# ofsoundof/GRL-Image-Restoration

Hardware: NVIDIA H100
Metric: Mpix/s (input pixels) GRL-Base x4 SR 256x256 tiles (higher is better)
Workload: dtype f16

## Files before the change

grl-image-restoration_b200/csrc/gemm_tc.cu:

```cuda
#include <algorithm>

#include "grl_common.cuh"
#include "tc_common.cuh"
#include "ops_tc.h"

namespace grl {
namespace tc {

EncodeTiledFn encode_tiled_fn() {
  static EncodeTiledFn fn = nullptr;
  if (!fn) {
    void* p = nullptr;
    cudaDriverEntryPointQueryResult q;
    if (cudaGetDriverEntryPoint("cuTensorMapEncodeTiled", &p, cudaEnableDefault, &q) == cudaSuccess &&
        q == cudaDriverEntryPointSuccess)
      fn = (EncodeTiledFn)p;
  }
  return fn;
}

__device__ __forceinline__ float gelu_as(float x) {
  const float z = fabsf(x) * 0.70710678118654752440f;
  float t, e;
  asm("rcp.approx.ftz.f32 %0, %1;" : "=f"(t) : "f"(fmaf(0.3275911f, z, 1.0f)));
  asm("ex2.approx.ftz.f32 %0, %1;" : "=f"(e) : "f"(-z * z * 1.4426950408889634f));
  float p = fmaf(1.061405429f, t, -1.453152027f);
  p = fmaf(p, t, 1.421413741f);
  p = fmaf(p, t, -0.284496736f);
  p = fmaf(p, t, 0.254829592f);
  const float erf_abs = fmaf(-p * t, e, 1.0f);
  const float half_x = 0.5f * x;
  return fmaf(half_x, copysignf(erf_abs, x), half_x);
}
__device__ __forceinline__ float tc_act(float v, int act, float slope) {
  if (act == GRL_ACT_GELU) return gelu_as(v);
  if (act == GRL_ACT_LEAKY) return v > 0.f ? v : v * slope;
  return v;
}

constexpr int kStages = 4;
constexpr int kBM = 128, kBK = 64;
constexpr int kTH = 8, kTW = 16;
constexpr int kEpiWarps = 8, kEpiThreads = kEpiWarps * 32, kThreads = kEpiThreads + 32;

__host__ __device__ constexpr int stage_pitch32(int c) { return (c % 8 == 4) ? c : ((c + 3) / 4 * 4 % 8 == 4 ? (c + 3) / 4 * 4 : (c + 3) / 4 * 4 + 4); }

template <int BN>
struct GemmSmem {
  static constexpr int A_BYTES = kBM * kBK * 2;
  static constexpr int B_BYTES = BN * kBK * 2;
  static constexpr int STAGE = A_BYTES + B_BYTES;
  static constexpr int PIPE = kStages * STAGE;
  static constexpr int AP = BN + 4;
  static constexpr int ACC = kBM * AP * 4;
  static constexpr int STG32 = kBM * stage_pitch32(BN <= 192 ? (BN == 192 ? 188 : BN) : 4) * 4;
  static constexpr int STG16 = kBM * (BN + 8) * 2;
  static constexpr int STG = (STG32 > STG16 ? STG32 : STG16);
  static constexpr int OFF_STG = ACC;
  static constexpr int OFF_TOK = ((PIPE > ACC + STG ? PIPE : ACC + STG) + 15) / 16 * 16;
  static constexpr int OFF_PAR = OFF_TOK + 128 * 8 + 128 * 4;
  static constexpr int OFF_MOM = OFF_PAR + 3 * BN * 4;
  static constexpr int OFF_BAR = OFF_MOM + 2 * 128 * 3 * 4;
  static constexpr int TOTAL = OFF_BAR + 128 + 1024 ;
  static_assert(AP % 8 == 4, "accumulator pitch");
  static_assert(TOTAL <= 232448, "shared memory budget");
};

__device__ __forceinline__ void epi_barrier() { asm volatile("bar.sync 1, 256;" ::: "memory"); }

__device__ __forceinline__ void acc_row32(const float* p, uint32_t (&v)[32]) {
#pragma unroll
  for (int j = 0; j < 32; j += 4) {
    const uint4 x = *reinterpret_cast<const uint4*>(p + j);
    v[j] = x.x, v[j + 1] = x.y, v[j + 2] = x.z, v[j + 3] = x.w;
  }
}

template <int BN, int FMT>
__device__ __forceinline__ void mma_loop(float (&acc)[BN / 64][32], uint8_t* smem, uint64_t* full, uint64_t* empty,
                                         int nk_total, int half, int et) {
  using S = GemmSmem<BN>;
  for (int kc = 0; kc < nk_total; ++kc) {
    const int s = kc % kStages;
    mbar_wait(&full[s], (kc / kStages) & 1);
    const uint32_t sa = smem_u32(smem + s * S::STAGE) + half * (64 * 128);
    const uint32_t sb = smem_u32(smem + s * S::STAGE + S::A_BYTES);
    wgmma_fence();
#pragma unroll
    for (int k = 0; k < kBK / 16; ++k) {
      const uint64_t ad = gmma_desc(sa + k * 32, 16, 1024, SWZ_128B);
#pragma unroll
      for (int j = 0; j < BN / 64; ++j) {
        const uint64_t bd = gmma_desc(sb + j * (64 * 128) + k * 32, 16, 1024, SWZ_128B);
        if (FMT == FMT_BF16) wgmma_n64_bf16(acc[j], ad, bd, true);
        else wgmma_n64_f16(acc[j], ad, bd, true);
      }
    }
    wgmma_commit();
    wgmma_wait<1>();
    if (kc > 0 && (et & 127) == 0) mbar_arrive(&empty[(kc - 1) % kStages]);
  }
  wgmma_wait<0>();
}

template <int BN, int EPI, bool CONV>
__global__ void __launch_bounds__(kThreads, 1)
gemm_tc_kernel(const __grid_constant__ CUtensorMap tmA, const __grid_constant__ CUtensorMap tmB, const GemmTcArgs a) {
  extern __shared__ uint8_t smem_raw[];
  uint8_t* smem = reinterpret_cast<uint8_t*>((reinterpret_cast<uintptr_t>(smem_raw) + 1023) & ~uintptr_t(1023));
  using S = GemmSmem<BN>;
  constexpr int AP = S::AP;
  uint64_t* full = reinterpret_cast<uint64_t*>(smem + S::OFF_BAR);
  uint64_t* empty = full + kStages;
  long long* s_tok = reinterpret_cast<long long*>(smem + S::OFF_TOK);
  int* s_img = reinterpret_cast<int*>(smem + S::OFF_TOK + 128 * 8);
  float* s_bias = reinterpret_cast<float*>(smem + S::OFF_PAR);
  float* s_gamma = s_bias + BN;
  float* s_beta = s_gamma + BN;
  float* s_mom = reinterpret_cast<float*>(smem + S::OFF_MOM);
  float* accs = reinterpret_cast<float*>(smem);

  const int warp = threadIdx.x >> 5, lane = threadIdx.x & 31;
  const int n_tiles = a.n_tiles;
  const int m_idx = blockIdx.x / n_tiles;
  const int n0 = (blockIdx.x - m_idx * n_tiles) * BN;
  const int nk_total = a.taps * a.nk;
  int m0 = 0, tb = 0, ty0 = 0, tx0 = 0;
  if (CONV) {
    int t = m_idx;
    const int tx = t % a.tiles_x;
    t /= a.tiles_x;
    const int ty = t % a.tiles_y;
    tb = t / a.tiles_y;
    ty0 = ty * kTH;
    tx0 = tx * kTW;
  } else {
    m0 = m_idx * kBM;
  }

  if (threadIdx.x == 0) {
    for (int s = 0; s < kStages; ++s) {
      mbar_init(&full[s], 1);
      mbar_init(&empty[s], 2);
    }
    mbar_init_fence();
    tma_prefetch_desc(&tmA);
    tma_prefetch_desc(&tmB);
  }
  __syncthreads();

  if (warp == kEpiWarps) {
    if (lane == 0) {
      for (int kc = 0; kc < nk_total; ++kc) {
        const int s = kc % kStages;
        mbar_wait(&empty[s], ((kc / kStages) & 1) ^ 1);
        uint8_t* sa = smem + s * S::STAGE;
        uint8_t* sb = sa + S::A_BYTES;
        mbar_expect_tx(&full[s], S::STAGE);
        if (CONV) {
          const int tap = kc / a.nk, c0 = (kc - tap * a.nk) * kBK;
          tma_load_4d(sa, &tmA, &full[s], c0, tx0 + (tap % 3) - 1, ty0 + (tap / 3) - 1, tb);
        } else {
          tma_load_2d(sa, &tmA, &full[s], kc * kBK, m0);
        }
        tma_load_2d(sb, &tmB, &full[s], kc * kBK, n0);
      }
    }
    return;
  }

  const int et = threadIdx.x;
  const int q = warp & 3;
  const int row = q * 32 + lane;
  const int half = et >> 7;
  const int fmt = a.fmt;
  uint16_t* out16 = reinterpret_cast<uint16_t*>(a.out_bf16);
  {
    long long tok;
    if (CONV) {
      const int y = ty0 + row / kTW, x = tx0 + row % kTW;
      tok = (y < a.H && x < a.W) ? ((long long)tb * a.H + y) * a.W + x : -1;
    } else {
      tok = (long long)m0 + row;
      if (tok >= a.M) tok = -1;
    }
    if (half == 0) {
      s_tok[row] = tok;
      s_img[row] = (EPI == EPI_LN && tok >= 0) ? (int)(tok / a.L) : 0;
    }
    for (int c = et; c < BN; c += kEpiThreads) {
      const int n = n0 + c;
      s_bias[c] = (n < a.N) ? a.bias[n] : 0.f;
      if (EPI == EPI_LN) {
        s_gamma[c] = (c < a.C) ? a.gamma[c] : 0.f;
        s_beta[c] = (c < a.C) ? a.beta[c] : 0.f;
      }
    }
  }
  {
    float acc[BN / 64][32];
#pragma unroll
    for (int j = 0; j < BN / 64; ++j)
#pragma unroll
      for (int e = 0; e < 32; ++e) acc[j][e] = 0.f;
    if (fmt == FMT_BF16) mma_loop<BN, FMT_BF16>(acc, smem, full, empty, nk_total, half, et);
    else mma_loop<BN, FMT_F16>(acc, smem, full, empty, nk_total, half, et);
    epi_barrier();
    const int w = (et >> 5) & 3, r0 = half * 64 + 16 * w + (lane >> 2), cq = 2 * (lane & 3);
#pragma unroll
    for (int j = 0; j < BN / 64; ++j)
#pragma unroll
      for (int i = 0; i < 8; ++i) {
        const int c = j * 64 + 8 * i + cq;
        *reinterpret_cast<float2*>(accs + r0 * AP + c) = make_float2(acc[j][4 * i], acc[j][4 * i + 1]);
        *reinterpret_cast<float2*>(accs + (r0 + 8) * AP + c) = make_float2(acc[j][4 * i + 2], acc[j][4 * i + 3]);
      }
  }
  epi_barrier();
  uint32_t v[32];

    if (EPI == EPI_BIAS_ACT && a.epi_mode == 2) {
      const long long tok = s_tok[row];
      for (int c0 = 32 * half; c0 < BN; c0 += 64) {
        if (n0 + c0 >= a.N) break;
        acc_row32(accs + row * AP + c0, v);
        if (tok < 0) continue;
        float o[32];
#pragma unroll
        for (int j = 0; j < 32; ++j) {
          const int n = n0 + c0 + j;
          float val = tc_act(__uint_as_float(v[j]) + s_bias[c0 + j], a.act, a.slope);
          if (a.res_f32 && n < a.N_f32) val += __ldg(a.res_f32 + tok * a.ldr + n);
          o[j] = (n < a.N) ? val : 0.f;
          if (a.out_f32 && n < a.N_f32) a.out_f32[tok * a.ldo_f32 + n] = o[j];
          if (CONV && a.out_nchw && n < a.N_f32) {
            const int r = a.nchw_r, rr = r * r;
            const int c = n / rr, q = n - c * rr;
            const int yy = (ty0 + row / kTW) * r + q / r, xx = (tx0 + row % kTW) * r + q % r;
            if (yy < a.Hc && xx < a.Wc)
              a.out_nchw[(((long long)tb * (a.N_f32 / rr) + c) * a.Hc + yy) * a.Wc + xx] = fmaf(o[j], a.post_scale, a.post_shift[c & 3]);
          }
        }
        if (out16) {
#pragma unroll
          for (int j = 0; j < 32; j += 8)
            if (n0 + c0 + j < a.ldo_bf16)
              *reinterpret_cast<uint4*>(out16 + tok * a.ldo_bf16 + n0 + c0 + j) =
                  make_uint4(pack16(o[j], o[j + 1], fmt), pack16(o[j + 2], o[j + 3], fmt), pack16(o[j + 4], o[j + 5], fmt),
                             pack16(o[j + 6], o[j + 7], fmt));
        }
      }
    } else if (a.epi_mode == 1) {
      const int Cw = (EPI == EPI_LN) ? a.C : a.N_f32;
      const int pitch = stage_pitch32(Cw);
      float* stg = reinterpret_cast<float*>(smem + S::OFF_STG);
      const bool res_in_stage = a.res_f32 != nullptr;
      if (res_in_stage) {
        const int C4r = Cw >> 2, ewr = et >> 5;
        for (int r = ewr; r < kBM; r += kEpiWarps) {
          const long long rtok = s_tok[r];
          for (int c4 = lane; c4 < C4r; c4 += 32)
            cp_async_16(stg + r * pitch + c4 * 4, a.res_f32 + (rtok >= 0 ? rtok : 0) * a.ldr + c4 * 4, rtok >= 0);
        }
        cp_async_commit();
      }
      if (EPI == EPI_LN) {
        float s1 = 0.f, s2 = 0.f, x0 = 0.f;
        int nh = 0;
        for (int c0 = 32 * half; c0 < Cw; c0 += 64) {
          acc_row32(accs + row * AP + c0, v);
          if (c0 == 32 * half) x0 = __uint_as_float(v[0]) + s_bias[c0];
#pragma unroll
          for (int j = 0; j < 32; ++j)
            if (c0 + j < Cw) {
              const float d = __uint_as_float(v[j]) + s_bias[c0 + j] - x0;
              s1 += d;
              s2 = fmaf(d, d, s2);
              ++nh;
            }
        }
        {
          const float fn = (float)nh;
          const float m1 = nh > 0 ? s1 / fn : 0.f;
          s_mom[(half * kBM + row) * 3 + 0] = x0 + m1;
          s_mom[(half * kBM + row) * 3 + 1] = nh > 0 ? fmaxf(s2 - s1 * m1, 0.f) : 0.f;
          s_mom[(half * kBM + row) * 3 + 2] = fn;
        }
        if (res_in_stage) cp_async_wait<0>();
        epi_barrier();
        float mean, rstd;
        {
          const float m0 = s_mom[row * 3 + 0], q0 = s_mom[row * 3 + 1], c0n = s_mom[row * 3 + 2];
          const float m1 = s_mom[(kBM + row) * 3 + 0], q1 = s_mom[(kBM + row) * 3 + 1], c1n = s_mom[(kBM + row) * 3 + 2];
          const float n = c0n + c1n, d = (c1n > 0.f) ? m1 - m0 : 0.f;
          mean = m0 + d * (c1n / n);
          const float M2 = q0 + q1 + d * d * (c0n * c1n / n);
          rstd = rsqrtf(M2 / n + a.eps);
        }
        for (int c0 = 32 * half; c0 < Cw; c0 += 64) {
          acc_row32(accs + row * AP + c0, v);
#pragma unroll
          for (int j = 0; j < 32; j += 4) {
            if (c0 + j < Cw) {
              float4* sp = reinterpret_cast<float4*>(stg + row * pitch + c0 + j);
              float4 acc4 = res_in_stage ? *sp : make_float4(0.f, 0.f, 0.f, 0.f);
              float o4[4] = {acc4.x, acc4.y, acc4.z, acc4.w};
#pragma unroll
              for (int e = 0; e < 4; ++e) {
                const int c = c0 + j + e;
                o4[e] += ((__uint_as_float(v[j + e]) + s_bias[c] - mean) * rstd * s_gamma[c] + s_beta[c]) * a.res_scale;
              }
              *sp = make_float4(o4[0], o4[1], o4[2], o4[3]);
            }
          }
        }
      } else {
        if (res_in_stage) {
          cp_async_wait<0>();
          epi_barrier();
        }
        for (int c0 = 32 * half; c0 < Cw; c0 += 64) {
          acc_row32(accs + row * AP + c0, v);
#pragma unroll
          for (int j = 0; j < 32; j += 4) {
            if (c0 + j < Cw) {
              float4* sp = reinterpret_cast<float4*>(stg + row * pitch + c0 + j);
              float4 acc4 = res_in_stage ? *sp : make_float4(0.f, 0.f, 0.f, 0.f);
              float o4[4] = {acc4.x, acc4.y, acc4.z, acc4.w};
#pragma unroll
              for (int e = 0; e < 4; ++e) o4[e] += tc_act(__uint_as_float(v[j + e]) + s_bias[c0 + j + e], a.act, a.slope);
              *sp = make_float4(o4[0], o4[1], o4[2], o4[3]);
            }
          }
        }
      }
      epi_barrier();
      const int C4 = Cw >> 2;
      const int P4 = out16 ? (int)(a.ldo_bf16 >> 2) : C4;
      const int ew = et >> 5;
      const bool has_cab = (EPI == EPI_LN) && a.cab_y != nullptr;
      const uint16_t* caby = reinterpret_cast<const uint16_t*>(a.cab_y);
      constexpr int RB = 8;
      for (int cbase = 0; cbase < P4; cbase += 32) {
        const int c4 = cbase + lane;
        const bool col_real = c4 < C4, col_any = c4 < P4;
        for (int rb = 0; rb < kBM / kEpiWarps; rb += RB) {
          long long tok[RB];
          float4 gg[RB];
          uint2 cy[RB];
#pragma unroll
          for (int i = 0; i < RB; ++i) {
            tok[i] = s_tok[ew + kEpiWarps * (rb + i)];
            gg[i] = make_float4(0.f, 0.f, 0.f, 0.f);
            cy[i] = make_uint2(0u, 0u);
            if (tok[i] >= 0 && col_real) {
              if (has_cab) {
                cy[i] = __ldg(reinterpret_cast<const uint2*>(caby + tok[i] * a.ld_caby + c4 * 4));
                gg[i] = __ldg(reinterpret_cast<const float4*>(a.cab_gate + (long long)s_img[ew + kEpiWarps * (rb + i)] * Cw + c4 * 4));
              }
            }
          }
#pragma unroll
          for (int i = 0; i < RB; ++i) {
            if (tok[i] < 0 || !col_any) continue;
            float4 val = make_float4(0.f, 0.f, 0.f, 0.f);
            if (col_real) {
              val = *reinterpret_cast<const float4*>(stg + (ew + kEpiWarps * (rb + i)) * pitch + c4 * 4);
              if (has_cab) {
                const float2 c01 = unpack16(cy[i].x, fmt), c23 = unpack16(cy[i].y, fmt);
                val.x = fmaf(c01.x, gg[i].x, val.x), val.y = fmaf(c01.y, gg[i].y, val.y);
                val.z = fmaf(c23.x, gg[i].z, val.z), val.w = fmaf(c23.y, gg[i].w, val.w);
              }
              if (a.out_f32) *reinterpret_cast<float4*>(a.out_f32 + tok[i] * a.ldo_f32 + c4 * 4) = val;
            }
            if (out16)
              *reinterpret_cast<uint2*>(out16 + tok[i] * a.ldo_bf16 + c4 * 4) =
                  make_uint2(pack16(val.x, val.y, fmt), pack16(val.z, val.w, fmt));
          }
        }
      }
    } else {
      constexpr int P16 = BN + 8;
      uint16_t* stg = reinterpret_cast<uint16_t*>(smem + S::OFF_STG);
      const int ncols = min(BN, a.N - n0);
      for (int c0 = 32 * half; c0 < ncols; c0 += 64) {
        acc_row32(accs + row * AP + c0, v);
        float o[32];
        if (EPI == EPI_QKV) {
          const int slot = (n0 + c0) >> 5;
          float ss = 0.f;
#pragma unroll
          for (int j = 0; j < 32; ++j) {
            o[j] = __uint_as_float(v[j]) + s_bias[c0 + j];
            ss = fmaf(o[j], o[j], ss);
          }
          const float sc = __ldg(a.slot_scale + slot);
          const float mul = sc > 0.f ? sc * rsqrtf(fmaxf(ss, 1e-24f)) : 1.0f;
#pragma unroll
          for (int j = 0; j < 32; ++j) o[j] *= mul;
        } else {
#pragma unroll
          for (int j = 0; j < 32; ++j) o[j] = tc_act(__uint_as_float(v[j]) + s_bias[c0 + j], a.act, a.slope);
        }
#pragma unroll
        for (int j = 0; j < 32; j += 8)
          *reinterpret_cast<uint4*>(stg + row * P16 + c0 + j) =
              make_uint4(pack16(o[j], o[j + 1], fmt), pack16(o[j + 2], o[j + 3], fmt), pack16(o[j + 4], o[j + 5], fmt),
                         pack16(o[j + 6], o[j + 7], fmt));
      }
      epi_barrier();
      const int nvec = min((long long)ncols, a.ldo_bf16 - n0) >> 3;
      const int ew = et >> 5;
      if (CONV && a.ps_r > 0) {
        const int ps = a.ps_r, Cq = a.N / (ps * ps);
        const int nv = min(BN, a.N - n0) >> 3;
#pragma unroll 4
        for (int r = ew; r < kBM; r += kEpiWarps) {
          if (s_tok[r] < 0) continue;
          const int y = ty0 + r / kTW, x = tx0 + r % kTW;
          for (int vv = lane; vv < nv; vv += 32) {
            const int n = n0 + vv * 8;
            const int q = n / Cq, c = n - q * Cq;
            const long long dtok = ((long long)tb * a.H * ps + y * ps + q / ps) * ((long long)a.W * ps) + x * ps + q % ps;
            *reinterpret_cast<uint4*>(out16 + dtok * a.ldo_bf16 + c) = *reinterpret_cast<const uint4*>(stg + r * P16 + vv * 8);
          }
        }
      } else {
#pragma unroll 4
        for (int r = ew; r < kBM; r += kEpiWarps) {
          const long long tok = s_tok[r];
          if (tok < 0) continue;
          for (int vv = lane; vv < nvec; vv += 32)
            *reinterpret_cast<uint4*>(out16 + tok * a.ldo_bf16 + n0 + vv * 8) = *reinterpret_cast<const uint4*>(stg + r * P16 + vv * 8);
        }
      }
    }

}

static int make_map(CUtensorMap* m, const void* base, int rank, const cuuint64_t* dims, const cuuint64_t* strides_bytes,
                    const cuuint32_t* box, int fmt) {
  EncodeTiledFn fn = encode_tiled_fn();
  if (!fn) return fail(GRL_ERR_CUDA, "cuTensorMapEncodeTiled is not available from the driver");
  cuuint32_t ones[5] = {1, 1, 1, 1, 1};
  CUresult rc = fn(m, fmt == FMT_BF16 ? CU_TENSOR_MAP_DATA_TYPE_BFLOAT16 : CU_TENSOR_MAP_DATA_TYPE_FLOAT16, (cuuint32_t)rank, const_cast<void*>(base), dims, strides_bytes,
                   box, ones, CU_TENSOR_MAP_INTERLEAVE_NONE, CU_TENSOR_MAP_SWIZZLE_128B,
                   CU_TENSOR_MAP_L2_PROMOTION_L2_128B, CU_TENSOR_MAP_FLOAT_OOB_FILL_NONE);
  if (rc != CUDA_SUCCESS) return fail(GRL_ERR_CUDA, "cuTensorMapEncodeTiled failed with CUresult %d", (int)rc);
  return GRL_OK;
}

template <int BN, int EPI, bool CONV>
static int launch_one(const CUtensorMap& tmA, const CUtensorMap& tmB, const GemmTcArgs& a, dim3 grid, cudaStream_t st) {
  auto kern = gemm_tc_kernel<BN, EPI, CONV>;
  static bool configured[kMaxDevices] = {false};
  int dev = 0;
  GRL_CUDA(cudaGetDevice(&dev));
  if (dev < 0 || dev >= kMaxDevices || !configured[dev]) {
    GRL_CUDA(cudaFuncSetAttribute(kern, cudaFuncAttributeMaxDynamicSharedMemorySize, GemmSmem<BN>::TOTAL));
    if (dev >= 0 && dev < kMaxDevices) configured[dev] = true;
  }
  kern<<<grid, kThreads, GemmSmem<BN>::TOTAL, st>>>(tmA, tmB, a);
  GRL_LAUNCH_CHECK("gemm_tc_kernel");
  return GRL_OK;
}

template <int EPI, bool CONV>
static int dispatch_bn(int bn, const CUtensorMap& tmA, const CUtensorMap& tmB, const GemmTcArgs& a, dim3 grid,
                       cudaStream_t st) {
  switch (bn) {
    case 64: return launch_one<64, EPI, CONV>(tmA, tmB, a, grid, st);
    case 128: return launch_one<128, EPI, CONV>(tmA, tmB, a, grid, st);
    case 192: return launch_one<192, EPI, CONV>(tmA, tmB, a, grid, st);
    case 256: return launch_one<256, EPI, CONV>(tmA, tmB, a, grid, st);
  }
  return fail(GRL_ERR_INVALID, "gemm_tc: unsupported tile width %d", bn);
}

int pick_bn(int npad) {
  if (npad <= 64) return 64;
  if (npad <= 128) return 128;
  if (npad % 192 == 0 || npad <= 192) return 192;
  if (npad % 256 == 0) return 256;
  return npad % 128 == 0 ? 128 : 192;
}

int plan_gemm_tc(const GemmTcProblem& p, GemmTcArgs& a, int* bn_out) {
  GRL_REQUIRE(p.kpad % kBK == 0 && p.kpad > 0, "gemm_tc: K pad %d must be a multiple of 64", p.kpad);
  GRL_REQUIRE(p.npad % 32 == 0 && p.npad > 0, "gemm_tc: N pad %d must be a multiple of 32", p.npad);
  int bn = (p.epi == EPI_LN) ? (p.npad <= 64 ? 64 : p.npad <= 128 ? 128 : p.npad <= 192 ? 192 : 256) : pick_bn(p.npad);
  GRL_REQUIRE(p.epi != EPI_LN || p.npad <= 256, "gemm_tc: LayerNorm epilogue needs the whole row in one tile (N=%d)",
              p.npad);
  const bool conv = p.taps == 9;
  if (a.ps_r > 0)
    GRL_REQUIRE(conv && p.epi == EPI_BIAS_ACT && !a.out_f32 && !a.res_f32 && a.out_bf16 && a.N % (a.ps_r * a.ps_r) == 0 &&
                    (a.N / (a.ps_r * a.ps_r)) % 8 == 0 && a.ldo_bf16 >= a.N / (a.ps_r * a.ps_r),
                "gemm_tc: pixel-shuffle store needs a 16-bit-only conv epilogue with N %% r^2 == 0 and N / r^2 %% 8 == 0");
  if (a.out_nchw)
    GRL_REQUIRE(conv && p.epi == EPI_BIAS_ACT && a.nchw_r >= 1 && a.N_f32 % (a.nchw_r * a.nchw_r) == 0 &&
                    a.N_f32 / (a.nchw_r * a.nchw_r) <= 4 && a.Hc > 0 && a.Wc > 0,
                "gemm_tc: NCHW tail store needs a conv with <= 4 output channels");
  GRL_REQUIRE(p.taps == 1 || p.taps == 9, "gemm_tc: taps must be 1 or 9");
  a.epi_mode = 0;
  if (p.epi == EPI_LN || (p.epi == EPI_BIAS_ACT && (a.out_f32 || a.res_f32))) {
    const int cw = p.epi == EPI_LN ? a.C : a.N_f32;
    const int cap = bn == 64 ? GemmSmem<64>::STG : bn == 128 ? GemmSmem<128>::STG : bn == 192 ? GemmSmem<192>::STG
                                                                                               : GemmSmem<256>::STG;
    const bool ok = p.npad <= bn && cw > 0 && cw % 4 == 0 && kBM * stage_pitch32(cw) * 4 <= cap &&
                    (!a.out_f32 || a.ldo_f32 % 4 == 0) && (!a.res_f32 || a.ldr % 4 == 0) &&
                    (!a.out_bf16 || a.ldo_bf16 % 4 == 0);
    GRL_REQUIRE(ok || p.epi != EPI_LN, "gemm_tc: LayerNorm epilogue needs C %% 4 == 0 and C <= 188 (got %d)", cw);
    a.epi_mode = ok ? 1 : 2;
  }
  if (a.out_nchw) a.epi_mode = 2;
  GRL_REQUIRE(p.epi == EPI_BIAS_ACT || p.epi == EPI_QKV || p.epi == EPI_LN, "gemm_tc: unknown epilogue %d", p.epi);
  GRL_REQUIRE(!conv || p.epi == EPI_BIAS_ACT, "gemm_tc: %s epilogue is linear-only", p.epi == EPI_QKV ? "QKV" : "LN");
  a.nk = p.kpad / kBK;
  a.taps = p.taps;
  a.n_tiles = ceil_div(p.npad, bn);
  if (conv) {
    a.H = p.H, a.W = p.W;
    a.tiles_x = ceil_div(p.W, kTW), a.tiles_y = ceil_div(p.H, kTH);
    a.M = (long long)p.B * p.H * p.W;
    GRL_REQUIRE((long long)a.tiles_x * a.tiles_y * p.B * a.n_tiles < (1ll << 31), "gemm_tc: grid too large");
    a.total_tiles = a.tiles_x * a.tiles_y * p.B * a.n_tiles;
  } else {
    a.M = p.M;
    GRL_REQUIRE((long long)ceil_div(p.M, kBM) * a.n_tiles < (1ll << 31), "gemm_tc: grid too large");
    a.total_tiles = (int)(ceil_div(p.M, kBM) * a.n_tiles);
  }
  *bn_out = bn;
  return GRL_OK;
}

int launch_gemm_tc(const GemmTcProblem& p, GemmTcArgs a, cudaStream_t st) {
  int bn = 0, rc;
  if ((rc = plan_gemm_tc(p, a, &bn)) != GRL_OK) return rc;
  if (a.M == 0) return GRL_OK;
  CUtensorMap tmA, tmB;
  if (p.taps == 9) {
    cuuint64_t dims[4] = {(cuuint64_t)p.kpad, (cuuint64_t)p.W, (cuuint64_t)p.H, (cuuint64_t)p.B};
    cuuint64_t str[3] = {(cuuint64_t)p.kpad * 2, (cuuint64_t)p.W * p.kpad * 2, (cuuint64_t)p.H * p.W * p.kpad * 2};
    cuuint32_t box[4] = {(cuuint32_t)kBK, (cuuint32_t)kTW, (cuuint32_t)kTH, 1};
    if ((rc = make_map(&tmA, p.x, 4, dims, str, box, a.fmt)) != GRL_OK) return rc;
  } else {
    cuuint64_t dims[2] = {(cuuint64_t)p.kpad, (cuuint64_t)p.M};
    cuuint64_t str[1] = {(cuuint64_t)p.kpad * 2};
    cuuint32_t box[2] = {(cuuint32_t)kBK, (cuuint32_t)kBM};
    if ((rc = make_map(&tmA, p.x, 2, dims, str, box, a.fmt)) != GRL_OK) return rc;
  }
  {
    cuuint64_t dims[2] = {(cuuint64_t)p.kpad * p.taps, (cuuint64_t)p.npad};
    cuuint64_t str[1] = {(cuuint64_t)p.kpad * p.taps * 2};
    cuuint32_t box[2] = {(cuuint32_t)kBK, (cuuint32_t)bn};
    if ((rc = make_map(&tmB, p.w, 2, dims, str, box, a.fmt)) != GRL_OK) return rc;
  }
  const dim3 grid((unsigned)a.total_tiles);
  switch (p.epi) {
    case EPI_QKV: return dispatch_bn<EPI_QKV, false>(bn, tmA, tmB, a, grid, st);
    case EPI_LN: return dispatch_bn<EPI_LN, false>(bn, tmA, tmB, a, grid, st);
  }
  return p.taps == 9 ? dispatch_bn<EPI_BIAS_ACT, true>(bn, tmA, tmB, a, grid, st)
                     : dispatch_bn<EPI_BIAS_ACT, false>(bn, tmA, tmB, a, grid, st);
}

}
}
```

grl-image-restoration_b200/csrc/tc_common.cuh:

```cuda
#pragma once
#include <cuda.h>
#include <cuda_bf16.h>
#include <cuda_fp16.h>
#include <cuda_runtime.h>
#include <stdint.h>

namespace grl {
namespace tc {

__device__ __forceinline__ uint32_t smem_u32(const void* p) { return (uint32_t)__cvta_generic_to_shared(p); }

__device__ __forceinline__ void mbar_init(uint64_t* bar, uint32_t count) {
  asm volatile("mbarrier.init.shared::cta.b64 [%0], %1;" ::"r"(smem_u32(bar)), "r"(count) : "memory");
}
__device__ __forceinline__ void mbar_init_fence() { asm volatile("fence.mbarrier_init.release.cluster;" ::: "memory"); }
__device__ __forceinline__ void mbar_expect_tx(uint64_t* bar, uint32_t bytes) {
  asm volatile("mbarrier.arrive.expect_tx.shared::cta.b64 _, [%0], %1;" ::"r"(smem_u32(bar)), "r"(bytes) : "memory");
}
__device__ __forceinline__ void mbar_arrive(uint64_t* bar) {
  asm volatile("mbarrier.arrive.shared::cta.b64 _, [%0];" ::"r"(smem_u32(bar)) : "memory");
}
__device__ __forceinline__ bool mbar_try_wait(uint64_t* bar, uint32_t parity) {
  uint32_t ok;
  asm volatile(
      "{\n\t.reg .pred p;\n\t"
      "mbarrier.try_wait.parity.shared::cta.b64 p, [%1], %2, %3;\n\t"
      "selp.u32 %0, 1, 0, p;\n\t}"
      : "=r"(ok)
      : "r"(smem_u32(bar)), "r"(parity), "r"(1000000u)
      : "memory");
  return ok != 0;
}
__device__ __forceinline__ void mbar_wait(uint64_t* bar, uint32_t parity) {
  if (mbar_try_wait(bar, parity)) return;
  int spins = 0;
  long long t0 = 0;
  while (!mbar_try_wait(bar, parity)) {
    if ((++spins & 63) == 0) {
      const long long now = clock64();
      if (t0 == 0) t0 = now;
      else if (now - t0 > 4000000000ll) __trap();
    }
  }
}

__device__ __forceinline__ void fence_proxy_async_smem() { asm volatile("fence.proxy.async.shared::cta;" ::: "memory"); }

__device__ __forceinline__ void tma_prefetch_desc(const CUtensorMap* m) {
  asm volatile("prefetch.tensormap [%0];" ::"l"(reinterpret_cast<uint64_t>(m)) : "memory");
}
__device__ __forceinline__ void tma_load_2d(void* smem, const CUtensorMap* m, uint64_t* bar, int c0, int c1) {
  asm volatile(
      "cp.async.bulk.tensor.2d.shared::cluster.global.mbarrier::complete_tx::bytes [%0], [%1, {%3, %4}], [%2];" ::"r"(
          smem_u32(smem)),
      "l"(reinterpret_cast<uint64_t>(m)), "r"(smem_u32(bar)), "r"(c0), "r"(c1)
      : "memory");
}
__device__ __forceinline__ void tma_load_4d(void* smem, const CUtensorMap* m, uint64_t* bar, int c0, int c1, int c2,
                                            int c3) {
  asm volatile(
      "cp.async.bulk.tensor.4d.shared::cluster.global.mbarrier::complete_tx::bytes [%0], [%1, {%3, %4, %5, %6}], "
      "[%2];" ::"r"(smem_u32(smem)),
      "l"(reinterpret_cast<uint64_t>(m)), "r"(smem_u32(bar)), "r"(c0), "r"(c1), "r"(c2), "r"(c3)
      : "memory");
}

__device__ __forceinline__ void cp_async_16(void* smem, const void* gmem, bool valid) {
  const int sz = valid ? 16 : 0;
  asm volatile("cp.async.cg.shared.global [%0], [%1], 16, %2;" ::"r"(smem_u32(smem)), "l"(gmem), "r"(sz) : "memory");
}
__device__ __forceinline__ void bulk_load_1d(void* smem, const void* gmem, uint32_t bytes, uint64_t* bar) {
  asm volatile("cp.async.bulk.shared::cluster.global.mbarrier::complete_tx::bytes [%0], [%1], %2, [%3];" ::"r"(smem_u32(smem)),
               "l"(gmem), "r"(bytes), "r"(smem_u32(bar))
               : "memory");
}
__device__ __forceinline__ void cp_async_commit() { asm volatile("cp.async.commit_group;" ::: "memory"); }
template <int N>
__device__ __forceinline__ void cp_async_wait() {
  asm volatile("cp.async.wait_group %0;" ::"n"(N) : "memory");
}

enum : uint32_t { SWZ_NONE = 0, SWZ_128B = 1, SWZ_64B = 2, SWZ_32B = 3 };
__device__ __forceinline__ uint64_t gmma_desc(uint32_t saddr, uint32_t lbo_bytes, uint32_t sbo_bytes, uint32_t swz) {
  uint64_t d = 0;
  d |= (uint64_t)((saddr & 0x3FFFFu) >> 4);
  d |= (uint64_t)((lbo_bytes >> 4) & 0x3FFFu) << 16;
  d |= (uint64_t)((sbo_bytes >> 4) & 0x3FFFu) << 32;
  d |= (uint64_t)swz << 62;
  return d;
}
__device__ __forceinline__ void wgmma_fence() { asm volatile("wgmma.fence.sync.aligned;" ::: "memory"); }
__device__ __forceinline__ void wgmma_commit() { asm volatile("wgmma.commit_group.sync.aligned;" ::: "memory"); }
template <int N>
__device__ __forceinline__ void wgmma_wait() {
  asm volatile("wgmma.wait_group.sync.aligned %0;" ::"n"(N) : "memory");
}
template <int N>
__device__ __forceinline__ void wgmma_fence_regs(float (&d)[N]) {
#pragma unroll
  for (int i = 0; i < N; ++i) asm volatile("" : "+f"(d[i])::"memory");
}
#define GRL_D16 "+f"(d[0]), "+f"(d[1]), "+f"(d[2]), "+f"(d[3]), "+f"(d[4]), "+f"(d[5]), "+f"(d[6]), "+f"(d[7]), "+f"(d[8]), "+f"(d[9]), "+f"(d[10]), "+f"(d[11]), "+f"(d[12]), "+f"(d[13]), "+f"(d[14]), "+f"(d[15])
#define GRL_D32 GRL_D16, "+f"(d[16]), "+f"(d[17]), "+f"(d[18]), "+f"(d[19]), "+f"(d[20]), "+f"(d[21]), "+f"(d[22]), "+f"(d[23]), "+f"(d[24]), "+f"(d[25]), "+f"(d[26]), "+f"(d[27]), "+f"(d[28]), "+f"(d[29]), "+f"(d[30]), "+f"(d[31])
#define GRL_R16 "%0, %1, %2, %3, %4, %5, %6, %7, %8, %9, %10, %11, %12, %13, %14, %15"
#define GRL_R32 GRL_R16 ", %16, %17, %18, %19, %20, %21, %22, %23, %24, %25, %26, %27, %28, %29, %30, %31"
#define GRL_WGMMA(NAME, N, NREG, REGS, OUTS, A, B, P, TY, TNSPB)                                                    \
  __device__ __forceinline__ void NAME(float (&d)[NREG], uint64_t adesc, uint64_t bdesc, bool accumulate) {         \
    asm volatile("{\n\t.reg .pred p;\n\tsetp.ne.b32 p, %" #P ", 0;\n\t"                                                 \
                 "wgmma.mma_async.sync.aligned.m64n" #N "k16.f32." TY "." TY " {" REGS "}, %" #A ", %" #B ", p, 1, 1, 0, " \
                 #TNSPB ";\n\t}"                                                                                     \
                 : OUTS                                                                                              \
                 : "l"(adesc), "l"(bdesc), "r"((uint32_t)accumulate));                                               \
  }
GRL_WGMMA(wgmma_n64_bf16, 64, 32, GRL_R32, GRL_D32, 32, 33, 34, "bf16", 0)
GRL_WGMMA(wgmma_n64_f16, 64, 32, GRL_R32, GRL_D32, 32, 33, 34, "f16", 0)
GRL_WGMMA(wgmma_n32t_bf16, 32, 16, GRL_R16, GRL_D16, 16, 17, 18, "bf16", 1)
GRL_WGMMA(wgmma_n32t_f16, 32, 16, GRL_R16, GRL_D16, 16, 17, 18, "f16", 1)
#define GRL_WGMMA_RS(NAME, TY)                                                                                        \
  __device__ __forceinline__ void NAME(float (&d)[16], const uint32_t (&a)[4], uint64_t bdesc) {                     \
    asm volatile("{\n\t.reg .pred p;\n\tsetp.ne.b32 p, 1, 0;\n\t"                                                    \
                 "wgmma.mma_async.sync.aligned.m64n32k16.f32." TY "." TY " {" GRL_R16 "}, {%16, %17, %18, %19}, %20, " \
                 "p, 1, 1, 1;\n\t}"                                                                                 \
                 : GRL_D16                                                                                          \
                 : "r"(a[0]), "r"(a[1]), "r"(a[2]), "r"(a[3]), "l"(bdesc));                                         \
  }
GRL_WGMMA_RS(wgmma_rs_n32t_bf16, "bf16")
GRL_WGMMA_RS(wgmma_rs_n32t_f16, "f16")

__device__ __forceinline__ uint32_t pack_bf16(float lo, float hi) {
  __nv_bfloat162 v = __floats2bfloat162_rn(lo, hi);
  return *reinterpret_cast<uint32_t*>(&v);
}
enum : int { FMT_F16 = 0, FMT_BF16 = 1 };
__device__ __forceinline__ uint32_t pack_f16(float lo, float hi) {
  uint32_t d;
  asm("cvt.rn.satfinite.f16x2.f32 %0, %1, %2;" : "=r"(d) : "f"(hi), "f"(lo));
  return d;
}
__device__ __forceinline__ uint32_t pack16(float lo, float hi, int fmt) {
  return fmt == FMT_BF16 ? pack_bf16(lo, hi) : pack_f16(lo, hi);
}
__device__ __forceinline__ float2 unpack16(uint32_t v, int fmt) {
  if (fmt == FMT_BF16) return make_float2(__uint_as_float(v << 16), __uint_as_float(v & 0xFFFF0000u));
  return __half22float2(*reinterpret_cast<const __half2*>(&v));
}
__device__ __forceinline__ float unpack16_one(uint16_t v, int fmt) {
  if (fmt == FMT_BF16) return __uint_as_float((uint32_t)v << 16);
  return __half2float(*reinterpret_cast<const __half*>(&v));
}

typedef CUresult (*EncodeTiledFn)(CUtensorMap*, CUtensorMapDataType, cuuint32_t, void*, const cuuint64_t*,
                                  const cuuint64_t*, const cuuint32_t*, const cuuint32_t*, CUtensorMapInterleave,
                                  CUtensorMapSwizzle, CUtensorMapL2promotion, CUtensorMapFloatOOBfill);
EncodeTiledFn encode_tiled_fn();

}
}
```

Before: 1.576.

## Make tensor-core GEMM persistent with wide WGMMA and register-resident epilogue

Turns the warp-specialized TMA/WGMMA GEMM into a persistent kernel that loops over tiles with a global pipeline iteration counter, so loads for the next tile overlap the current tile's epilogue. Single wide m64nBNk16 WGMMA instructions (N=128/192/256) replace multiple n64 issues. The epilogue works directly from registers instead of staging the fp32 accumulator tile through shared memory, and computes LayerNorm statistics with warp shuffles and Chan merging. The freed shared memory allows per-BN stage counts, cp.async prefetch of the residual and two CTAs per SM for BN=64. The risks are higher register pressure from the wide accumulators and more complex barrier phase tracking.

Measured after the change: 1.627 (median of 6 runs). 1.03x the previous value.

```diff
diff --git a/grl-image-restoration_b200/csrc/gemm_tc.cu b/grl-image-restoration_b200/csrc/gemm_tc.cu
--- a/grl-image-restoration_b200/csrc/gemm_tc.cu
+++ b/grl-image-restoration_b200/csrc/gemm_tc.cu
@@ -38,7 +38,6 @@
   return v;
 }
 
-constexpr int kStages = 4;
 constexpr int kBM = 128, kBK = 64;
 constexpr int kTH = 8, kTW = 16;
 constexpr int kEpiWarps = 8, kEpiThreads = kEpiWarps * 32, kThreads = kEpiThreads + 32;
@@ -47,99 +46,132 @@
 
 template <int BN>
 struct GemmSmem {
+  static constexpr int STAGES = (BN >= 192 || BN == 64) ? 3 : 4;
   static constexpr int A_BYTES = kBM * kBK * 2;
   static constexpr int B_BYTES = BN * kBK * 2;
   static constexpr int STAGE = A_BYTES + B_BYTES;
-  static constexpr int PIPE = kStages * STAGE;
-  static constexpr int AP = BN + 4;
-  static constexpr int ACC = kBM * AP * 4;
+  static constexpr int PIPE = STAGES * STAGE;
   static constexpr int STG32 = kBM * stage_pitch32(BN <= 192 ? (BN == 192 ? 188 : BN) : 4) * 4;
   static constexpr int STG16 = kBM * (BN + 8) * 2;
   static constexpr int STG = (STG32 > STG16 ? STG32 : STG16);
-  static constexpr int OFF_STG = ACC;
-  static constexpr int OFF_TOK = ((PIPE > ACC + STG ? PIPE : ACC + STG) + 15) / 16 * 16;
+  static constexpr int OFF_STG = PIPE;
+  static constexpr int OFF_TOK = OFF_STG + STG;
   static constexpr int OFF_PAR = OFF_TOK + 128 * 8 + 128 * 4;
-  static constexpr int OFF_MOM = OFF_PAR + 3 * BN * 4;
-  static constexpr int OFF_BAR = OFF_MOM + 2 * 128 * 3 * 4;
-  static constexpr int TOTAL = OFF_BAR + 128 + 1024 ;
-  static_assert(AP % 8 == 4, "accumulator pitch");
+  static constexpr int OFF_BAR = OFF_PAR + 3 * BN * 4;
+  static constexpr int TOTAL = OFF_BAR + 2 * STAGES * 8 + 1024 ;
+  static_assert(STG % 16 == 0, "staging alignment");
   static_assert(TOTAL <= 232448, "shared memory budget");
 };
 
 __device__ __forceinline__ void epi_barrier() { asm volatile("bar.sync 1, 256;" ::: "memory"); }
 
-__device__ __forceinline__ void acc_row32(const float* p, uint32_t (&v)[32]) {
-#pragma unroll
-  for (int j = 0; j < 32; j += 4) {
-    const uint4 x = *reinterpret_cast<const uint4*>(p + j);
-    v[j] = x.x, v[j + 1] = x.y, v[j + 2] = x.z, v[j + 3] = x.w;
-  }
+struct TileCoord {
+  int n0, m0, tb, ty0, tx0;
+};
+template <int BN, bool CONV>
+__device__ __forceinline__ TileCoord tile_coord(const GemmTcArgs& a, int tile) {
+  TileCoord t{};
+  const int m_idx = tile / a.n_tiles;
+  t.n0 = (tile - m_idx * a.n_tiles) * BN;
+  if (CONV) {
+    int u = m_idx;
+    const int tx = u % a.tiles_x;
+    u /= a.tiles_x;
+    const int ty = u % a.tiles_y;
+    t.tb = u / a.tiles_y;
+    t.ty0 = ty * kTH;
+    t.tx0 = tx * kTW;
+  } else {
+    t.m0 = m_idx * kBM;
+  }
+  return t;
+}
+template <bool CONV>
+__device__ __forceinline__ long long row_token(const GemmTcArgs& a, const TileCoord& t, int r) {
+  if (CONV) {
+    const int y = t.ty0 + r / kTW, x = t.tx0 + r % kTW;
+    return (y < a.H && x < a.W) ? ((long long)t.tb * a.H + y) * a.W + x : -1;
+  }
+  const long long tok = (long long)t.m0 + r;
+  return tok < a.M ? tok : -1;
+}
+
+__device__ __forceinline__ void chan_merge(float& m0, float& q0, float& n0, float m1, float q1, float n1) {
+  if (n1 > 0.f) {
+    const float n = n0 + n1, d = m1 - m0;
+    m0 = m0 + d * (n1 / n);
+    q0 = q0 + q1 + d * d * (n0 * n1 / n);
+    n0 = n;
+  }
+}
+
+template <int BN>
+__device__ __forceinline__ void wgmma_wide_f16(float (&d)[BN / 64][32], uint64_t ad, uint64_t bd) {
+  if constexpr (BN == 128) wgmma_n128_f16(d, ad, bd);
+  else if constexpr (BN == 192) wgmma_n192_f16(d, ad, bd);
+  else if constexpr (BN == 256) wgmma_n256_f16(d, ad, bd);
+}
+template <int BN>
+__device__ __forceinline__ void wgmma_wide_bf16(float (&d)[BN / 64][32], uint64_t ad, uint64_t bd) {
+  if constexpr (BN == 128) wgmma_n128_bf16(d, ad, bd);
+  else if constexpr (BN == 192) wgmma_n192_bf16(d, ad, bd);
+  else if constexpr (BN == 256) wgmma_n256_bf16(d, ad, bd);
 }
 
 template <int BN, int FMT>
 __device__ __forceinline__ void mma_loop(float (&acc)[BN / 64][32], uint8_t* smem, uint64_t* full, uint64_t* empty,
-                                         int nk_total, int half, int et) {
+                                         uint32_t it, int nk_total, int half, int et) {
   using S = GemmSmem<BN>;
   for (int kc = 0; kc < nk_total; ++kc) {
-    const int s = kc % kStages;
-    mbar_wait(&full[s], (kc / kStages) & 1);
+    const uint32_t g = it + kc;
+    const int s = g % S::STAGES;
+    mbar_wait(&full[s], (g / S::STAGES) & 1);
     const uint32_t sa = smem_u32(smem + s * S::STAGE) + half * (64 * 128);
     const uint32_t sb = smem_u32(smem + s * S::STAGE + S::A_BYTES);
     wgmma_fence();
 #pragma unroll
     for (int k = 0; k < kBK / 16; ++k) {
       const uint64_t ad = gmma_desc(sa + k * 32, 16, 1024, SWZ_128B);
-#pragma unroll
-      for (int j = 0; j < BN / 64; ++j) {
-        const uint64_t bd = gmma_desc(sb + j * (64 * 128) + k * 32, 16, 1024, SWZ_128B);
-        if (FMT == FMT_BF16) wgmma_n64_bf16(acc[j], ad, bd, true);
-        else wgmma_n64_f16(acc[j], ad, bd, true);
+      const uint64_t bd = gmma_desc(sb + k * 32, 16, 1024, SWZ_128B);
+      if (BN == 64) {
+        if (FMT == FMT_BF16) wgmma_n64_bf16(acc[0], ad, bd, true);
+        else wgmma_n64_f16(acc[0], ad, bd, true);
+      } else if (FMT == FMT_BF16) {
+        wgmma_wide_bf16<BN>(acc, ad, bd);
+      } else {
+        wgmma_wide_f16<BN>(acc, ad, bd);
       }
     }
     wgmma_commit();
     wgmma_wait<1>();
-    if (kc > 0 && (et & 127) == 0) mbar_arrive(&empty[(kc - 1) % kStages]);
+    if (kc > 0 && (et & 127) == 0) mbar_arrive(&empty[(g - 1) % S::STAGES]);
   }
   wgmma_wait<0>();
+  if ((et & 127) == 0) mbar_arrive(&empty[(it + nk_total - 1) % S::STAGES]);
+#pragma unroll
+  for (int j = 0; j < BN / 64; ++j) wgmma_fence_regs(acc[j]);
 }
 
 template <int BN, int EPI, bool CONV>
-__global__ void __launch_bounds__(kThreads, 1)
+__global__ void __launch_bounds__(kThreads, (BN == 64 && EPI != EPI_LN) ? 2 : 1)
 gemm_tc_kernel(const __grid_constant__ CUtensorMap tmA, const __grid_constant__ CUtensorMap tmB, const GemmTcArgs a) {
   extern __shared__ uint8_t smem_raw[];
   uint8_t* smem = reinterpret_cast<uint8_t*>((reinterpret_cast<uintptr_t>(smem_raw) + 1023) & ~uintptr_t(1023));
   using S = GemmSmem<BN>;
-  constexpr int AP = S::AP;
+  constexpr int NS = S::STAGES;
   uint64_t* full = reinterpret_cast<uint64_t*>(smem + S::OFF_BAR);
-  uint64_t* empty = full + kStages;
+  uint64_t* empty = full + NS;
   long long* s_tok = reinterpret_cast<long long*>(smem + S::OFF_TOK);
   int* s_img = reinterpret_cast<int*>(smem + S::OFF_TOK + 128 * 8);
   float* s_bias = reinterpret_cast<float*>(smem + S::OFF_PAR);
   float* s_gamma = s_bias + BN;
   float* s_beta = s_gamma + BN;
-  float* s_mom = reinterpret_cast<float*>(smem + S::OFF_MOM);
-  float* accs = reinterpret_cast<float*>(smem);
 
   const int warp = threadIdx.x >> 5, lane = threadIdx.x & 31;
-  const int n_tiles = a.n_tiles;
-  const int m_idx = blockIdx.x / n_tiles;
-  const int n0 = (blockIdx.x - m_idx * n_tiles) * BN;
   const int nk_total = a.taps * a.nk;
-  int m0 = 0, tb = 0, ty0 = 0, tx0 = 0;
-  if (CONV) {
-    int t = m_idx;
-    const int tx = t % a.tiles_x;
-    t /= a.tiles_x;
-    const int ty = t % a.tiles_y;
-    tb = t / a.tiles_y;
-    ty0 = ty * kTH;
-    tx0 = tx * kTW;
-  } else {
-    m0 = m_idx * kBM;
-  }
 
   if (threadIdx.x == 0) {
-    for (int s = 0; s < kStages; ++s) {
+    for (int s = 0; s < NS; ++s) {
       mbar_init(&full[s], 1);
       mbar_init(&empty[s], 2);
     }
@@ -147,192 +179,191 @@
     tma_prefetch_desc(&tmA);
     tma_prefetch_desc(&tmB);
   }
+  if (EPI == EPI_LN)
+    for (int c = threadIdx.x; c < BN; c += kThreads) {
+      s_gamma[c] = (c < a.C) ? a.gamma[c] : 0.f;
+      s_beta[c] = (c < a.C) ? a.beta[c] : 0.f;
+    }
   __syncthreads();
 
   if (warp == kEpiWarps) {
     if (lane == 0) {
-      for (int kc = 0; kc < nk_total; ++kc) {
-        const int s = kc % kStages;
-        mbar_wait(&empty[s], ((kc / kStages) & 1) ^ 1);
-        uint8_t* sa = smem + s * S::STAGE;
-        uint8_t* sb = sa + S::A_BYTES;
-        mbar_expect_tx(&full[s], S::STAGE);
-        if (CONV) {
-          const int tap = kc / a.nk, c0 = (kc - tap * a.nk) * kBK;
-          tma_load_4d(sa, &tmA, &full[s], c0, tx0 + (tap % 3) - 1, ty0 + (tap / 3) - 1, tb);
-        } else {
-          tma_load_2d(sa, &tmA, &full[s], kc * kBK, m0);
+      uint32_t it = 0;
+      for (int tile = blockIdx.x; tile < a.total_tiles; tile += gridDim.x) {
+        const TileCoord t = tile_coord<BN, CONV>(a, tile);
+        for (int kc = 0; kc < nk_total; ++kc, ++it) {
+          const int s = it % NS;
+          mbar_wait(&empty[s], ((it / NS) & 1) ^ 1);
+          uint8_t* sa = smem + s * S::STAGE;
+          uint8_t* sb = sa + S::A_BYTES;
+          mbar_expect_tx(&full[s], S::STAGE);
+          if (CONV) {
+            const int tap = kc / a.nk, c0 = (kc - tap * a.nk) * kBK;
+            tma_load_4d(sa, &tmA, &full[s], c0, t.tx0 + (tap % 3) - 1, t.ty0 + (tap / 3) - 1, t.tb);
+          } else {
+            tma_load_2d(sa, &tmA, &full[s], kc * kBK, t.m0);
+          }
+          tma_load_2d(sb, &tmB, &full[s], kc * kBK, t.n0);
         }
-        tma_load_2d(sb, &tmB, &full[s], kc * kBK, n0);
       }
     }
     return;
   }
 
   const int et = threadIdx.x;
-  const int q = warp & 3;
-  const int row = q * 32 + lane;
   const int half = et >> 7;
+  const int rA = half * 64 + 16 * ((et >> 5) & 3) + (lane >> 2), cq = 2 * (lane & 3);
   const int fmt = a.fmt;
   uint16_t* out16 = reinterpret_cast<uint16_t*>(a.out_bf16);
-  {
-    long long tok;
-    if (CONV) {
-      const int y = ty0 + row / kTW, x = tx0 + row % kTW;
-      tok = (y < a.H && x < a.W) ? ((long long)tb * a.H + y) * a.W + x : -1;
-    } else {
-      tok = (long long)m0 + row;
-      if (tok >= a.M) tok = -1;
-    }
-    if (half == 0) {
-      s_tok[row] = tok;
-      s_img[row] = (EPI == EPI_LN && tok >= 0) ? (int)(tok / a.L) : 0;
-    }
-    for (int c = et; c < BN; c += kEpiThreads) {
-      const int n = n0 + c;
-      s_bias[c] = (n < a.N) ? a.bias[n] : 0.f;
+  const int Cw = (EPI == EPI_LN) ? a.C : a.N_f32;
+  const int pitch = stage_pitch32(Cw);
+  const bool res_in_stage = a.epi_mode == 1 && a.res_f32 != nullptr;
+  float* stg32 = reinterpret_cast<float*>(smem + S::OFF_STG);
+  constexpr int P16 = BN + 8;
+  uint16_t* stg16 = reinterpret_cast<uint16_t*>(smem + S::OFF_STG);
+  uint32_t it = 0;
+  int bias_n0 = -1;
+
+  for (int tile = blockIdx.x; tile < a.total_tiles; tile += gridDim.x, it += nk_total) {
+    const TileCoord t = tile_coord<BN, CONV>(a, tile);
+    if (et < kBM) {
+      const long long tok = row_token<CONV>(a, t, et);
+      s_tok[et] = tok;
+      s_img[et] = (EPI == EPI_LN && tok >= 0) ? (int)(tok / a.L) : 0;
+    }
+    if (t.n0 != bias_n0) {
+      for (int c = et; c < BN; c += kEpiThreads) s_bias[c] = (t.n0 + c < a.N) ? a.bias[t.n0 + c] : 0.f;
+      bias_n0 = t.n0;
+    }
+    if (res_in_stage) {
+      const int C4r = Cw >> 2;
+      for (int r = et >> 5; r < kBM; r += kEpiWarps) {
+        const long long rtok = row_token<CONV>(a, t, r);
+        for (int c4 = lane; c4 < C4r; c4 += 32)
+          cp_async_16(stg32 + r * pitch + c4 * 4, a.res_f32 + (rtok >= 0 ? rtok : 0) * a.ldr + c4 * 4, rtok >= 0);
+      }
+      cp_async_commit();
+    }
+    float acc[BN / 64][32];
+#pragma unroll
+    for (int j = 0; j < BN / 64; ++j)
+#pragma unroll
+      for (int e = 0; e < 32; ++e) acc[j][e] = 0.f;
+    if (fmt == FMT_BF16) mma_loop<BN, FMT_BF16>(acc, smem, full, empty, it, nk_total, half, et);
+    else mma_loop<BN, FMT_F16>(acc, smem, full, empty, it, nk_total, half, et);
+    if (res_in_stage) cp_async_wait<0>();
+    epi_barrier();
+
+    if (BN <= 192 && EPI == EPI_BIAS_ACT && a.epi_mode == 2) {
+      long long tokr[2] = {row_token<CONV>(a, t, rA), row_token<CONV>(a, t, rA + 8)};
+#pragma unroll
+      for (int j = 0; j < BN / 64; ++j)
+#pragma unroll
+        for (int i = 0; i < 8; ++i) {
+          const int c = 64 * j + 8 * i + cq;
+          if (t.n0 + (c & ~31) >= a.N) continue;
+#pragma unroll
+          for (int h = 0; h < 2; ++h) {
+            const long long tok = tokr[h];
+            if (tok < 0) continue;
+            const int row = rA + 8 * h;
+            float o[2];
+#pragma unroll
+            for (int e = 0; e < 2; ++e) {
+              const int n = t.n0 + c + e;
+              float val = tc_act(acc[j][4 * i + 2 * h + e] + s_bias[c + e], a.act, a.slope);
+              if (a.res_f32 && n < a.N_f32) val += __ldg(a.res_f32 + tok * a.ldr + n);
+              o[e] = (n < a.N) ? val : 0.f;
+              if (a.out_f32 && n < a.N_f32) a.out_f32[tok * a.ldo_f32 + n] = o[e];
+              if (CONV && a.out_nchw && n < a.N_f32) {
+                const int r = a.nchw_r, rr = r * r;
+                const int ch = n / rr, q = n - ch * rr;
+                const int yy = (t.ty0 + row / kTW) * r + q / r, xx = (t.tx0 + row % kTW) * r + q % r;
+                if (yy < a.Hc && xx < a.Wc)
+                  a.out_nchw[(((long long)t.tb * (a.N_f32 / rr) + ch) * a.Hc + yy) * a.Wc + xx] =
+                      fmaf(o[e], a.post_scale, a.post_shift[ch & 3]);
+              }
+            }
+            if (out16 && t.n0 + (c & ~7) < a.ldo_bf16)
+              *reinterpret_cast<uint32_t*>(out16 + tok * a.ldo_bf16 + t.n0 + c) = pack16(o[0], o[1], fmt);
+          }
+        }
+      epi_barrier();
+      continue;
+    }
+    if (BN <= 192 && a.epi_mode == 1) {
       if (EPI == EPI_LN) {
-        s_gamma[c] = (c < a.C) ? a.gamma[c] : 0.f;
-        s_beta[c] = (c < a.C) ? a.beta[c] : 0.f;
-      }
-    }
-  }
-  {
-    float acc[BN / 64][32];
-#pragma unroll
-    for (int j = 0; j < BN / 64; ++j)
-#pragma unroll
-      for (int e = 0; e < 32; ++e) acc[j][e] = 0.f;
-    if (fmt == FMT_BF16) mma_loop<BN, FMT_BF16>(acc, smem, full, empty, nk_total, half, et);
-    else mma_loop<BN, FMT_F16>(acc, smem, full, empty, nk_total, half, et);
-    epi_barrier();
-    const int w = (et >> 5) & 3, r0 = half * 64 + 16 * w + (lane >> 2), cq = 2 * (lane & 3);
-#pragma unroll
-    for (int j = 0; j < BN / 64; ++j)
-#pragma unroll
-      for (int i = 0; i < 8; ++i) {
-        const int c = j * 64 + 8 * i + cq;
-        *reinterpret_cast<float2*>(accs + r0 * AP + c) = make_float2(acc[j][4 * i], acc[j][4 * i + 1]);
-        *reinterpret_cast<float2*>(accs + (r0 + 8) * AP + c) = make_float2(acc[j][4 * i + 2], acc[j][4 * i + 3]);
-      }
-  }
-  epi_barrier();
-  uint32_t v[32];
-
-    if (EPI == EPI_BIAS_ACT && a.epi_mode == 2) {
-      const long long tok = s_tok[row];
-      for (int c0 = 32 * half; c0 < BN; c0 += 64) {
-        if (n0 + c0 >= a.N) break;
-        acc_row32(accs + row * AP + c0, v);
-        if (tok < 0) continue;
-        float o[32];
-#pragma unroll
-        for (int j = 0; j < 32; ++j) {
-          const int n = n0 + c0 + j;
-          float val = tc_act(__uint_as_float(v[j]) + s_bias[c0 + j], a.act, a.slope);
-          if (a.res_f32 && n < a.N_f32) val += __ldg(a.res_f32 + tok * a.ldr + n);
-          o[j] = (n < a.N) ? val : 0.f;
-          if (a.out_f32 && n < a.N_f32) a.out_f32[tok * a.ldo_f32 + n] = o[j];
-          if (CONV && a.out_nchw && n < a.N_f32) {
-            const int r = a.nchw_r, rr = r * r;
-            const int c = n / rr, q = n - c * rr;
-            const int yy = (ty0 + row / kTW) * r + q / r, xx = (tx0 + row % kTW) * r + q % r;
-            if (yy < a.Hc && xx < a.Wc)
-              a.out_nchw[(((long long)tb * (a.N_f32 / rr) + c) * a.Hc + yy) * a.Wc + xx] = fmaf(o[j], a.post_scale, a.post_shift[c & 3]);
-          }
+        float mean[2], rstd[2];
+#pragma unroll
+        for (int h = 0; h < 2; ++h) {
+          const float x0 = acc[0][2 * h] + s_bias[cq];
+          float s1 = 0.f, s2 = 0.f;
+          int nh = 0;
+#pragma unroll
+          for (int j = 0; j < BN / 64; ++j)
+#pragma unroll
+            for (int i = 0; i < 8; ++i)
+#pragma unroll
+              for (int e = 0; e < 2; ++e) {
+                const int c = 64 * j + 8 * i + cq + e;
+                if (c < Cw) {
+                  const float d = acc[j][4 * i + 2 * h + e] + s_bias[c] - x0;
+                  s1 += d;
+                  s2 = fmaf(d, d, s2);
+                  ++nh;
+                }
+              }
+          float n = (float)nh;
+          const float m1 = nh > 0 ? s1 / n : 0.f;
+          float m = nh > 0 ? x0 + m1 : 0.f;
+          float q = nh > 0 ? fmaxf(s2 - s1 * m1, 0.f) : 0.f;
+#pragma unroll
+          for (int x = 1; x <= 2; x <<= 1) {
+            const float mo = __shfl_xor_sync(0xffffffffu, m, x), qo = __shfl_xor_sync(0xffffffffu, q, x),
+                        no = __shfl_xor_sync(0xffffffffu, n, x);
+            if (lane & x) {
+              float m2 = mo, q2 = qo, n2 = no;
+              chan_merge(m2, q2, n2, m, q, n);
+              m = m2, q = q2, n = n2;
+            } else {
+              chan_merge(m, q, n, mo, qo, no);
+            }
+          }
+          mean[h] = m;
+          rstd[h] = rsqrtf(q / n + a.eps);
         }
-        if (out16) {
-#pragma unroll
-          for (int j = 0; j < 32; j += 8)
-            if (n0 + c0 + j < a.ldo_bf16)
-              *reinterpret_cast<uint4*>(out16 + tok * a.ldo_bf16 + n0 + c0 + j) =
-                  make_uint4(pack16(o[j], o[j + 1], fmt), pack16(o[j + 2], o[j + 3], fmt), pack16(o[j + 4], o[j + 5], fmt),
-                             pack16(o[j + 6], o[j + 7], fmt));
-        }
-      }
-    } else if (a.epi_mode == 1) {
-      const int Cw = (EPI == EPI_LN) ? a.C : a.N_f32;
-      const int pitch = stage_pitch32(Cw);
-      float* stg = reinterpret_cast<float*>(smem + S::OFF_STG);
-      const bool res_in_stage = a.res_f32 != nullptr;
-      if (res_in_stage) {
-        const int C4r = Cw >> 2, ewr = et >> 5;
-        for (int r = ewr; r < kBM; r += kEpiWarps) {
-          const long long rtok = s_tok[r];
-          for (int c4 = lane; c4 < C4r; c4 += 32)
-            cp_async_16(stg + r * pitch + c4 * 4, a.res_f32 + (rtok >= 0 ? rtok : 0) * a.ldr + c4 * 4, rtok >= 0);
-        }
-        cp_async_commit();
-      }
-      if (EPI == EPI_LN) {
-        float s1 = 0.f, s2 = 0.f, x0 = 0.f;
-        int nh = 0;
-        for (int c0 = 32 * half; c0 < Cw; c0 += 64) {
-          acc_row32(accs + row * AP + c0, v);
-          if (c0 == 32 * half) x0 = __uint_as_float(v[0]) + s_bias[c0];
-#pragma unroll
-          for (int j = 0; j < 32; ++j)
-            if (c0 + j < Cw) {
-              const float d = __uint_as_float(v[j]) + s_bias[c0 + j] - x0;
-              s1 += d;
-              s2 = fmaf(d, d, s2);
-              ++nh;
+#pragma unroll
+        for (int j = 0; j < BN / 64; ++j)
+#pragma unroll
+          for (int i = 0; i < 8; ++i) {
+            const int c = 64 * j + 8 * i + cq;
+            if (c >= Cw) continue;
+#pragma unroll
+            for (int h = 0; h < 2; ++h) {
+              float2* sp = reinterpret_cast<float2*>(stg32 + (rA + 8 * h) * pitch + c);
+              float2 o = res_in_stage ? *sp : make_float2(0.f, 0.f);
+              o.x += ((acc[j][4 * i + 2 * h] + s_bias[c] - mean[h]) * rstd[h] * s_gamma[c] + s_beta[c]) * a.res_scale;
+              o.y += ((acc[j][4 * i + 2 * h + 1] + s_bias[c + 1] - mean[h]) * rstd[h] * s_gamma[c + 1] + s_beta[c + 1]) *
+                     a.res_scale;
+              *sp = o;
             }
-        }
-        {
-          const float fn = (float)nh;
-          const float m1 = nh > 0 ? s1 / fn : 0.f;
-          s_mom[(half * kBM + row) * 3 + 0] = x0 + m1;
-          s_mom[(half * kBM + row) * 3 + 1] = nh > 0 ? fmaxf(s2 - s1 * m1, 0.f) : 0.f;
-          s_mom[(half * kBM + row) * 3 + 2] = fn;
-        }
-        if (res_in_stage) cp_async_wait<0>();
-        epi_barrier();
-        float mean, rstd;
-        {
-          const float m0 = s_mom[row * 3 + 0], q0 = s_mom[row * 3 + 1], c0n = s_mom[row * 3 + 2];
-          const float m1 = s_mom[(kBM + row) * 3 + 0], q1 = s_mom[(kBM + row) * 3 + 1], c1n = s_mom[(kBM + row) * 3 + 2];
-          const float n = c0n + c1n, d = (c1n > 0.f) ? m1 - m0 : 0.f;
-          mean = m0 + d * (c1n / n);
-          const float M2 = q0 + q1 + d * d * (c0n * c1n / n);
-          rstd = rsqrtf(M2 / n + a.eps);
-        }
-        for (int c0 = 32 * half; c0 < Cw; c0 += 64) {
-          acc_row32(accs + row * AP + c0, v);
-#pragma unroll
-          for (int j = 0; j < 32; j += 4) {
-            if (c0 + j < Cw) {
-              float4* sp = reinterpret_cast<float4*>(stg + row * pitch + c0 + j);
-              float4 acc4 = res_in_stage ? *sp : make_float4(0.f, 0.f, 0.f, 0.f);
-              float o4[4] = {acc4.x, acc4.y, acc4.z, acc4.w};
-#pragma unroll
-              for (int e = 0; e < 4; ++e) {
-                const int c = c0 + j + e;
-                o4[e] += ((__uint_as_float(v[j + e]) + s_bias[c] - mean) * rstd * s_gamma[c] + s_beta[c]) * a.res_scale;
-              }
-              *sp = make_float4(o4[0], o4[1], o4[2], o4[3]);
+          }
+      } else {
+#pragma unroll
+        for (int j = 0; j < BN / 64; ++j)
+#pragma unroll
+          for (int i = 0; i < 8; ++i) {
+            const int c = 64 * j + 8 * i + cq;
+            if (c >= Cw) continue;
+#pragma unroll
+            for (int h = 0; h < 2; ++h) {
+              float2* sp = reinterpret_cast<float2*>(stg32 + (rA + 8 * h) * pitch + c);
+              float2 o = res_in_stage ? *sp : make_float2(0.f, 0.f);
+              o.x += tc_act(acc[j][4 * i + 2 * h] + s_bias[c], a.act, a.slope);
+              o.y += tc_act(acc[j][4 * i + 2 * h + 1] + s_bias[c + 1], a.act, a.slope);
+              *sp = o;
             }
           }
-        }
-      } else {
-        if (res_in_stage) {
-          cp_async_wait<0>();
-          epi_barrier();
-        }
-        for (int c0 = 32 * half; c0 < Cw; c0 += 64) {
-          acc_row32(accs + row * AP + c0, v);
-#pragma unroll
-          for (int j = 0; j < 32; j += 4) {
-            if (c0 + j < Cw) {
-              float4* sp = reinterpret_cast<float4*>(stg + row * pitch + c0 + j);
-              float4 acc4 = res_in_stage ? *sp : make_float4(0.f, 0.f, 0.f, 0.f);
-              float o4[4] = {acc4.x, acc4.y, acc4.z, acc4.w};
-#pragma unroll
-              for (int e = 0; e < 4; ++e) o4[e] += tc_act(__uint_as_float(v[j + e]) + s_bias[c0 + j + e], a.act, a.slope);
-              *sp = make_float4(o4[0], o4[1], o4[2], o4[3]);
-            }
-          }
-        }
       }
       epi_barrier();
       const int C4 = Cw >> 2;
@@ -365,7 +396,7 @@
             if (tok[i] < 0 || !col_any) continue;
             float4 val = make_float4(0.f, 0.f, 0.f, 0.f);
             if (col_real) {
-              val = *reinterpret_cast<const float4*>(stg + (ew + kEpiWarps * (rb + i)) * pitch + c4 * 4);
+              val = *reinterpret_cast<const float4*>(stg32 + (ew + kEpiWarps * (rb + i)) * pitch + c4 * 4);
               if (has_cab) {
                 const float2 c01 = unpack16(cy[i].x, fmt), c23 = unpack16(cy[i].y, fmt);
                 val.x = fmaf(c01.x, gg[i].x, val.x), val.y = fmaf(c01.y, gg[i].y, val.y);
@@ -380,49 +411,59 @@
         }
       }
     } else {
-      constexpr int P16 = BN + 8;
-      uint16_t* stg = reinterpret_cast<uint16_t*>(smem + S::OFF_STG);
-      const int ncols = min(BN, a.N - n0);
-      for (int c0 = 32 * half; c0 < ncols; c0 += 64) {
-        acc_row32(accs + row * AP + c0, v);
-        float o[32];
-        if (EPI == EPI_QKV) {
-          const int slot = (n0 + c0) >> 5;
-          float ss = 0.f;
-#pragma unroll
-          for (int j = 0; j < 32; ++j) {
-            o[j] = __uint_as_float(v[j]) + s_bias[c0 + j];
-            ss = fmaf(o[j], o[j], ss);
-          }
-          const float sc = __ldg(a.slot_scale + slot);
-          const float mul = sc > 0.f ? sc * rsqrtf(fmaxf(ss, 1e-24f)) : 1.0f;
-#pragma unroll
-          for (int j = 0; j < 32; ++j) o[j] *= mul;
-        } else {
-#pragma unroll
-          for (int j = 0; j < 32; ++j) o[j] = tc_act(__uint_as_float(v[j]) + s_bias[c0 + j], a.act, a.slope);
+      const int ncols = min(BN, a.N - t.n0);
+#pragma unroll
+      for (int j = 0; j < BN / 64; ++j)
+#pragma unroll
+        for (int s32 = 0; s32 < 2; ++s32) {
+          const int c0 = 64 * j + 32 * s32;
+          if (c0 >= ncols) continue;
+          float o[2][8];
+#pragma unroll
+          for (int h = 0; h < 2; ++h)
+#pragma unroll
+            for (int ii = 0; ii < 4; ++ii)
+#pragma unroll
+              for (int e = 0; e < 2; ++e) {
+                const float v = acc[j][4 * (4 * s32 + ii) + 2 * h + e] + s_bias[c0 + 8 * ii + cq + e];
+                o[h][2 * ii + e] = (EPI == EPI_QKV) ? v : tc_act(v, a.act, a.slope);
+              }
+          if (EPI == EPI_QKV) {
+            const float sc = __ldg(a.slot_scale + ((t.n0 + c0) >> 5));
+#pragma unroll
+            for (int h = 0; h < 2; ++h) {
+              float ss = 0.f;
+#pragma unroll
+              for (int k = 0; k < 8; ++k) ss = fmaf(o[h][k], o[h][k], ss);
+              ss += __shfl_xor_sync(0xffffffffu, ss, 1);
+              ss += __shfl_xor_sync(0xffffffffu, ss, 2);
+              const float mul = sc > 0.f ? sc * rsqrtf(fmaxf(ss, 1e-24f)) : 1.0f;
+#pragma unroll
+              for (int k = 0; k < 8; ++k) o[h][k] *= mul;
+            }
+          }
+#pragma unroll
+          for (int h = 0; h < 2; ++h)
+#pragma unroll
+            for (int ii = 0; ii < 4; ++ii)
+              *reinterpret_cast<uint32_t*>(stg16 + (rA + 8 * h) * P16 + c0 + 8 * ii + cq) =
+                  pack16(o[h][2 * ii], o[h][2 * ii + 1], fmt);
         }
-#pragma unroll
-        for (int j = 0; j < 32; j += 8)
-          *reinterpret_cast<uint4*>(stg + row * P16 + c0 + j) =
-              make_uint4(pack16(o[j], o[j + 1], fmt), pack16(o[j + 2], o[j + 3], fmt), pack16(o[j + 4], o[j + 5], fmt),
-                         pack16(o[j + 6], o[j + 7], fmt));
-      }
       epi_barrier();
-      const int nvec = min((long long)ncols, a.ldo_bf16 - n0) >> 3;
+      const int nvec = min((long long)ncols, a.ldo_bf16 - t.n0) >> 3;
       const int ew = et >> 5;
       if (CONV && a.ps_r > 0) {
         const int ps = a.ps_r, Cq = a.N / (ps * ps);
-        const int nv = min(BN, a.N - n0) >> 3;
+        const int nv = ncols >> 3;
 #pragma unroll 4
         for (int r = ew; r < kBM; r += kEpiWarps) {
           if (s_tok[r] < 0) continue;
-          const int y = ty0 + r / kTW, x = tx0 + r % kTW;
+          const int y = t.ty0 + r / kTW, x = t.tx0 + r % kTW;
           for (int vv = lane; vv < nv; vv += 32) {
-            const int n = n0 + vv * 8;
+            const int n = t.n0 + vv * 8;
             const int q = n / Cq, c = n - q * Cq;
-            const long long dtok = ((long long)tb * a.H * ps + y * ps + q / ps) * ((long long)a.W * ps) + x * ps + q % ps;
-            *reinterpret_cast<uint4*>(out16 + dtok * a.ldo_bf16 + c) = *reinterpret_cast<const uint4*>(stg + r * P16 + vv * 8);
+            const long long dtok = ((long long)t.tb * a.H * ps + y * ps + q / ps) * ((long long)a.W * ps) + x * ps + q % ps;
+            *reinterpret_cast<uint4*>(out16 + dtok * a.ldo_bf16 + c) = *reinterpret_cast<const uint4*>(stg16 + r * P16 + vv * 8);
           }
         }
       } else {
@@ -431,11 +472,12 @@
           const long long tok = s_tok[r];
           if (tok < 0) continue;
           for (int vv = lane; vv < nvec; vv += 32)
-            *reinterpret_cast<uint4*>(out16 + tok * a.ldo_bf16 + n0 + vv * 8) = *reinterpret_cast<const uint4*>(stg + r * P16 + vv * 8);
+            *reinterpret_cast<uint4*>(out16 + tok * a.ldo_bf16 + t.n0 + vv * 8) = *reinterpret_cast<const uint4*>(stg16 + r * P16 + vv * 8);
         }
       }
     }
-
+    epi_barrier();
+  }
 }
 
 static int make_map(CUtensorMap* m, const void* base, int rank, const cuuint64_t* dims, const cuuint64_t* strides_bytes,
@@ -450,29 +492,43 @@
   return GRL_OK;
 }
 
+static int sm_count(int dev) {
+  static int sms[kMaxDevices] = {0};
+  if (dev >= 0 && dev < kMaxDevices && sms[dev] > 0) return sms[dev];
+  int n = 0;
+  if (cudaDeviceGetAttribute(&n, cudaDevAttrMultiProcessorCount, dev) != cudaSuccess || n <= 0) return 0;
+  if (dev >= 0 && dev < kMaxDevices) sms[dev] = n;
+  return n;
+}
+
 template <int BN, int EPI, bool CONV>
-static int launch_one(const CUtensorMap& tmA, const CUtensorMap& tmB, const GemmTcArgs& a, dim3 grid, cudaStream_t st) {
+static int launch_one(const CUtensorMap& tmA, const CUtensorMap& tmB, const GemmTcArgs& a, cudaStream_t st) {
   auto kern = gemm_tc_kernel<BN, EPI, CONV>;
-  static bool configured[kMaxDevices] = {false};
+  static int resident[kMaxDevices] = {0};
   int dev = 0;
   GRL_CUDA(cudaGetDevice(&dev));
-  if (dev < 0 || dev >= kMaxDevices || !configured[dev]) {
+  int per_sm = (dev >= 0 && dev < kMaxDevices) ? resident[dev] : 0;
+  if (per_sm == 0) {
     GRL_CUDA(cudaFuncSetAttribute(kern, cudaFuncAttributeMaxDynamicSharedMemorySize, GemmSmem<BN>::TOTAL));
-    if (dev >= 0 && dev < kMaxDevices) configured[dev] = true;
-  }
+    GRL_CUDA(cudaOccupancyMaxActiveBlocksPerMultiprocessor(&per_sm, kern, kThreads, GemmSmem<BN>::TOTAL));
+    if (per_sm <= 0) return fail(GRL_ERR_CUDA, "gemm_tc: kernel does not fit on an SM of device %d", dev);
+    if (dev >= 0 && dev < kMaxDevices) resident[dev] = per_sm;
+  }
+  const int sms = sm_count(dev);
+  if (sms <= 0) return fail(GRL_ERR_CUDA, "gemm_tc: cannot read the SM count of device %d", dev);
+  const dim3 grid((unsigned)std::min((long long)a.total_tiles, (long long)sms * per_sm));
   kern<<<grid, kThreads, GemmSmem<BN>::TOTAL, st>>>(tmA, tmB, a);
   GRL_LAUNCH_CHECK("gemm_tc_kernel");
   return GRL_OK;
 }
 
 template <int EPI, bool CONV>
-static int dispatch_bn(int bn, const CUtensorMap& tmA, const CUtensorMap& tmB, const GemmTcArgs& a, dim3 grid,
-                       cudaStream_t st) {
+static int dispatch_bn(int bn, const CUtensorMap& tmA, const CUtensorMap& tmB, const GemmTcArgs& a, cudaStream_t st) {
   switch (bn) {
-    case 64: return launch_one<64, EPI, CONV>(tmA, tmB, a, grid, st);
-    case 128: return launch_one<128, EPI, CONV>(tmA, tmB, a, grid, st);
-    case 192: return launch_one<192, EPI, CONV>(tmA, tmB, a, grid, st);
-    case 256: return launch_one<256, EPI, CONV>(tmA, tmB, a, grid, st);
+    case 64: return launch_one<64, EPI, CONV>(tmA, tmB, a, st);
+    case 128: return launch_one<128, EPI, CONV>(tmA, tmB, a, st);
+    case 192: return launch_one<192, EPI, CONV>(tmA, tmB, a, st);
+    case 256: return launch_one<256, EPI, CONV>(tmA, tmB, a, st);
   }
   return fail(GRL_ERR_INVALID, "gemm_tc: unsupported tile width %d", bn);
 }
@@ -488,9 +544,10 @@
 int plan_gemm_tc(const GemmTcProblem& p, GemmTcArgs& a, int* bn_out) {
   GRL_REQUIRE(p.kpad % kBK == 0 && p.kpad > 0, "gemm_tc: K pad %d must be a multiple of 64", p.kpad);
   GRL_REQUIRE(p.npad % 32 == 0 && p.npad > 0, "gemm_tc: N pad %d must be a multiple of 32", p.npad);
-  int bn = (p.epi == EPI_LN) ? (p.npad <= 64 ? 64 : p.npad <= 128 ? 128 : p.npad <= 192 ? 192 : 256) : pick_bn(p.npad);
-  GRL_REQUIRE(p.epi != EPI_LN || p.npad <= 256, "gemm_tc: LayerNorm epilogue needs the whole row in one tile (N=%d)",
+  int bn = (p.epi == EPI_LN) ? (p.npad <= 64 ? 64 : p.npad <= 128 ? 128 : 192) : pick_bn(p.npad);
+  GRL_REQUIRE(p.epi != EPI_LN || p.npad <= 192, "gemm_tc: LayerNorm epilogue needs the whole row in one tile (N=%d)",
               p.npad);
+  if (bn == 256 && p.epi == EPI_BIAS_ACT && (a.out_f32 || a.res_f32 || a.out_nchw)) bn = 128;
   const bool conv = p.taps == 9;
   if (a.ps_r > 0)
     GRL_REQUIRE(conv && p.epi == EPI_BIAS_ACT && !a.out_f32 && !a.res_f32 && a.out_bf16 && a.N % (a.ps_r * a.ps_r) == 0 &&
@@ -555,14 +612,13 @@
     cuuint32_t box[2] = {(cuuint32_t)kBK, (cuuint32_t)bn};
     if ((rc = make_map(&tmB, p.w, 2, dims, str, box, a.fmt)) != GRL_OK) return rc;
   }
-  const dim3 grid((unsigned)a.total_tiles);
   switch (p.epi) {
-    case EPI_QKV: return dispatch_bn<EPI_QKV, false>(bn, tmA, tmB, a, grid, st);
-    case EPI_LN: return dispatch_bn<EPI_LN, false>(bn, tmA, tmB, a, grid, st);
-  }
-  return p.taps == 9 ? dispatch_bn<EPI_BIAS_ACT, true>(bn, tmA, tmB, a, grid, st)
-                     : dispatch_bn<EPI_BIAS_ACT, false>(bn, tmA, tmB, a, grid, st);
-}
-
-}
-}
+    case EPI_QKV: return dispatch_bn<EPI_QKV, false>(bn, tmA, tmB, a, st);
+    case EPI_LN: return dispatch_bn<EPI_LN, false>(bn, tmA, tmB, a, st);
+  }
+  return p.taps == 9 ? dispatch_bn<EPI_BIAS_ACT, true>(bn, tmA, tmB, a, st)
+                     : dispatch_bn<EPI_BIAS_ACT, false>(bn, tmA, tmB, a, st);
+}
+
+}
+}
diff --git a/grl-image-restoration_b200/csrc/tc_common.cuh b/grl-image-restoration_b200/csrc/tc_common.cuh
--- a/grl-image-restoration_b200/csrc/tc_common.cuh
+++ b/grl-image-restoration_b200/csrc/tc_common.cuh
@@ -124,6 +124,36 @@
                  : GRL_D16                                                                                          \
                  : "r"(a[0]), "r"(a[1]), "r"(a[2]), "r"(a[3]), "l"(bdesc));                                         \
   }
+__device__ __forceinline__ void wgmma_n128_f16(float (&d)[2][32], uint64_t adesc, uint64_t bdesc) {
+  asm volatile("{\n\t.reg .pred p;\n\tsetp.ne.b32 p, 1, 0;\n\twgmma.mma_async.sync.aligned.m64n128k16.f32.f16.f16 {%0, %1, %2, %3, %4, %5, %6, %7, %8, %9, %10, %11, %12, %13, %14, %15, %16, %17, %18, %19, %20, %21, %22, %23, %24, %25, %26, %27, %28, %29, %30, %31, %32, %33, %34, %35, %36, %37, %38, %39, %40, %41, %42, %43, %44, %45, %46, %47, %48, %49, %50, %51, %52, %53, %54, %55, %56, %57, %58, %59, %60, %61, %62, %63}, %64, %65, p, 1, 1, 0, 0;\n\t}"
+               : "+f"(d[0][0]), "+f"(d[0][1]), "+f"(d[0][2]), "+f"(d[0][3]), "+f"(d[0][4]), "+f"(d[0][5]), "+f"(d[0][6]), "+f"(d[0][7]), "+f"(d[0][8]), "+f"(d[0][9]), "+f"(d[0][10]), "+f"(d[0][11]), "+f"(d[0][12]), "+f"(d[0][13]), "+f"(d[0][14]), "+f"(d[0][15]), "+f"(d[0][16]), "+f"(d[0][17]), "+f"(d[0][18]), "+f"(d[0][19]), "+f"(d[0][20]), "+f"(d[0][21]), "+f"(d[0][22]), "+f"(d[0][23]), "+f"(d[0][24]), "+f"(d[0][25]), "+f"(d[0][26]), "+f"(d[0][27]), "+f"(d[0][28]), "+f"(d[0][29]), "+f"(d[0][30]), "+f"(d[0][31]), "+f"(d[1][0]), "+f"(d[1][1]), "+f"(d[1][2]), "+f"(d[1][3]), "+f"(d[1][4]), "+f"(d[1][5]), "+f"(d[1][6]), "+f"(d[1][7]), "+f"(d[1][8]), "+f"(d[1][9]), "+f"(d[1][10]), "+f"(d[1][11]), "+f"(d[1][12]), "+f"(d[1][13]), "+f"(d[1][14]), "+f"(d[1][15]), "+f"(d[1][16]), "+f"(d[1][17]), "+f"(d[1][18]), "+f"(d[1][19]), "+f"(d[1][20]), "+f"(d[1][21]), "+f"(d[1][22]), "+f"(d[1][23]), "+f"(d[1][24]), "+f"(d[1][25]), "+f"(d[1][26]), "+f"(d[1][27]), "+f"(d[1][28]), "+f"(d[1][29]), "+f"(d[1][30]), "+f"(d[1][31])
+               : "l"(adesc), "l"(bdesc));
+}
+__device__ __forceinline__ void wgmma_n128_bf16(float (&d)[2][32], uint64_t adesc, uint64_t bdesc) {
+  asm volatile("{\n\t.reg .pred p;\n\tsetp.ne.b32 p, 1, 0;\n\twgmma.mma_async.sync.aligned.m64n128k16.f32.bf16.bf16 {%0, %1, %2, %3, %4, %5, %6, %7, %8, %9, %10, %11, %12, %13, %14, %15, %16, %17, %18, %19, %20, %21, %22, %23, %24, %25, %26, %27, %28, %29, %30, %31, %32, %33, %34, %35, %36, %37, %38, %39, %40, %41, %42, %43, %44, %45, %46, %47, %48, %49, %50, %51, %52, %53, %54, %55, %56, %57, %58, %59, %60, %61, %62, %63}, %64, %65, p, 1, 1, 0, 0;\n\t}"
+               : "+f"(d[0][0]), "+f"(d[0][1]), "+f"(d[0][2]), "+f"(d[0][3]), "+f"(d[0][4]), "+f"(d[0][5]), "+f"(d[0][6]), "+f"(d[0][7]), "+f"(d[0][8]), "+f"(d[0][9]), "+f"(d[0][10]), "+f"(d[0][11]), "+f"(d[0][12]), "+f"(d[0][13]), "+f"(d[0][14]), "+f"(d[0][15]), "+f"(d[0][16]), "+f"(d[0][17]), "+f"(d[0][18]), "+f"(d[0][19]), "+f"(d[0][20]), "+f"(d[0][21]), "+f"(d[0][22]), "+f"(d[0][23]), "+f"(d[0][24]), "+f"(d[0][25]), "+f"(d[0][26]), "+f"(d[0][27]), "+f"(d[0][28]), "+f"(d[0][29]), "+f"(d[0][30]), "+f"(d[0][31]), "+f"(d[1][0]), "+f"(d[1][1]), "+f"(d[1][2]), "+f"(d[1][3]), "+f"(d[1][4]), "+f"(d[1][5]), "+f"(d[1][6]), "+f"(d[1][7]), "+f"(d[1][8]), "+f"(d[1][9]), "+f"(d[1][10]), "+f"(d[1][11]), "+f"(d[1][12]), "+f"(d[1][13]), "+f"(d[1][14]), "+f"(d[1][15]), "+f"(d[1][16]), "+f"(d[1][17]), "+f"(d[1][18]), "+f"(d[1][19]), "+f"(d[1][20]), "+f"(d[1][21]), "+f"(d[1][22]), "+f"(d[1][23]), "+f"(d[1][24]), "+f"(d[1][25]), "+f"(d[1][26]), "+f"(d[1][27]), "+f"(d[1][28]), "+f"(d[1][29]), "+f"(d[1][30]), "+f"(d[1][31])
+               : "l"(adesc), "l"(bdesc));
+}
+__device__ __forceinline__ void wgmma_n192_f16(float (&d)[3][32], uint64_t adesc, uint64_t bdesc) {
+  asm volatile("{\n\t.reg .pred p;\n\tsetp.ne.b32 p, 1, 0;\n\twgmma.mma_async.sync.aligned.m64n192k16.f32.f16.f16 {%0, %1, %2, %3, %4, %5, %6, %7, %8, %9, %10, %11, %12, %13, %14, %15, %16, %17, %18, %19, %20, %21, %22, %23, %24, %25, %26, %27, %28, %29, %30, %31, %32, %33, %34, %35, %36, %37, %38, %39, %40, %41, %42, %43, %44, %45, %46, %47, %48, %49, %50, %51, %52, %53, %54, %55, %56, %57, %58, %59, %60, %61, %62, %63, %64, %65, %66, %67, %68, %69, %70, %71, %72, %73, %74, %75, %76, %77, %78, %79, %80, %81, %82, %83, %84, %85, %86, %87, %88, %89, %90, %91, %92, %93, %94, %95}, %96, %97, p, 1, 1, 0, 0;\n\t}"
+               : "+f"(d[0][0]), "+f"(d[0][1]), "+f"(d[0][2]), "+f"(d[0][3]), "+f"(d[0][4]), "+f"(d[0][5]), "+f"(d[0][6]), "+f"(d[0][7]), "+f"(d[0][8]), "+f"(d[0][9]), "+f"(d[0][10]), "+f"(d[0][11]), "+f"(d[0][12]), "+f"(d[0][13]), "+f"(d[0][14]), "+f"(d[0][15]), "+f"(d[0][16]), "+f"(d[0][17]), "+f"(d[0][18]), "+f"(d[0][19]), "+f"(d[0][20]), "+f"(d[0][21]), "+f"(d[0][22]), "+f"(d[0][23]), "+f"(d[0][24]), "+f"(d[0][25]), "+f"(d[0][26]), "+f"(d[0][27]), "+f"(d[0][28]), "+f"(d[0][29]), "+f"(d[0][30]), "+f"(d[0][31]), "+f"(d[1][0]), "+f"(d[1][1]), "+f"(d[1][2]), "+f"(d[1][3]), "+f"(d[1][4]), "+f"(d[1][5]), "+f"(d[1][6]), "+f"(d[1][7]), "+f"(d[1][8]), "+f"(d[1][9]), "+f"(d[1][10]), "+f"(d[1][11]), "+f"(d[1][12]), "+f"(d[1][13]), "+f"(d[1][14]), "+f"(d[1][15]), "+f"(d[1][16]), "+f"(d[1][17]), "+f"(d[1][18]), "+f"(d[1][19]), "+f"(d[1][20]), "+f"(d[1][21]), "+f"(d[1][22]), "+f"(d[1][23]), "+f"(d[1][24]), "+f"(d[1][25]), "+f"(d[1][26]), "+f"(d[1][27]), "+f"(d[1][28]), "+f"(d[1][29]), "+f"(d[1][30]), "+f"(d[1][31]), "+f"(d[2][0]), "+f"(d[2][1]), "+f"(d[2][2]), "+f"(d[2][3]), "+f"(d[2][4]), "+f"(d[2][5]), "+f"(d[2][6]), "+f"(d[2][7]), "+f"(d[2][8]), "+f"(d[2][9]), "+f"(d[2][10]), "+f"(d[2][11]), "+f"(d[2][12]), "+f"(d[2][13]), "+f"(d[2][14]), "+f"(d[2][15]), "+f"(d[2][16]), "+f"(d[2][17]), "+f"(d[2][18]), "+f"(d[2][19]), "+f"(d[2][20]), "+f"(d[2][21]), "+f"(d[2][22]), "+f"(d[2][23]), "+f"(d[2][24]), "+f"(d[2][25]), "+f"(d[2][26]), "+f"(d[2][27]), "+f"(d[2][28]), "+f"(d[2][29]), "+f"(d[2][30]), "+f"(d[2][31])
+               : "l"(adesc), "l"(bdesc));
+}
+__device__ __forceinline__ void wgmma_n192_bf16(float (&d)[3][32], uint64_t adesc, uint64_t bdesc) {
+  asm volatile("{\n\t.reg .pred p;\n\tsetp.ne.b32 p, 1, 0;\n\twgmma.mma_async.sync.aligned.m64n192k16.f32.bf16.bf16 {%0, %1, %2, %3, %4, %5, %6, %7, %8, %9, %10, %11, %12, %13, %14, %15, %16, %17, %18, %19, %20, %21, %22, %23, %24, %25, %26, %27, %28, %29, %30, %31, %32, %33, %34, %35, %36, %37, %38, %39, %40, %41, %42, %43, %44, %45, %46, %47, %48, %49, %50, %51, %52, %53, %54, %55, %56, %57, %58, %59, %60, %61, %62, %63, %64, %65, %66, %67, %68, %69, %70, %71, %72, %73, %74, %75, %76, %77, %78, %79, %80, %81, %82, %83, %84, %85, %86, %87, %88, %89, %90, %91, %92, %93, %94, %95}, %96, %97, p, 1, 1, 0, 0;\n\t}"
+               : "+f"(d[0][0]), "+f"(d[0][1]), "+f"(d[0][2]), "+f"(d[0][3]), "+f"(d[0][4]), "+f"(d[0][5]), "+f"(d[0][6]), "+f"(d[0][7]), "+f"(d[0][8]), "+f"(d[0][9]), "+f"(d[0][10]), "+f"(d[0][11]), "+f"(d[0][12]), "+f"(d[0][13]), "+f"(d[0][14]), "+f"(d[0][15]), "+f"(d[0][16]), "+f"(d[0][17]), "+f"(d[0][18]), "+f"(d[0][19]), "+f"(d[0][20]), "+f"(d[0][21]), "+f"(d[0][22]), "+f"(d[0][23]), "+f"(d[0][24]), "+f"(d[0][25]), "+f"(d[0][26]), "+f"(d[0][27]), "+f"(d[0][28]), "+f"(d[0][29]), "+f"(d[0][30]), "+f"(d[0][31]), "+f"(d[1][0]), "+f"(d[1][1]), "+f"(d[1][2]), "+f"(d[1][3]), "+f"(d[1][4]), "+f"(d[1][5]), "+f"(d[1][6]), "+f"(d[1][7]), "+f"(d[1][8]), "+f"(d[1][9]), "+f"(d[1][10]), "+f"(d[1][11]), "+f"(d[1][12]), "+f"(d[1][13]), "+f"(d[1][14]), "+f"(d[1][15]), "+f"(d[1][16]), "+f"(d[1][17]), "+f"(d[1][18]), "+f"(d[1][19]), "+f"(d[1][20]), "+f"(d[1][21]), "+f"(d[1][22]), "+f"(d[1][23]), "+f"(d[1][24]), "+f"(d[1][25]), "+f"(d[1][26]), "+f"(d[1][27]), "+f"(d[1][28]), "+f"(d[1][29]), "+f"(d[1][30]), "+f"(d[1][31]), "+f"(d[2][0]), "+f"(d[2][1]), "+f"(d[2][2]), "+f"(d[2][3]), "+f"(d[2][4]), "+f"(d[2][5]), "+f"(d[2][6]), "+f"(d[2][7]), "+f"(d[2][8]), "+f"(d[2][9]), "+f"(d[2][10]), "+f"(d[2][11]), "+f"(d[2][12]), "+f"(d[2][13]), "+f"(d[2][14]), "+f"(d[2][15]), "+f"(d[2][16]), "+f"(d[2][17]), "+f"(d[2][18]), "+f"(d[2][19]), "+f"(d[2][20]), "+f"(d[2][21]), "+f"(d[2][22]), "+f"(d[2][23]), "+f"(d[2][24]), "+f"(d[2][25]), "+f"(d[2][26]), "+f"(d[2][27]), "+f"(d[2][28]), "+f"(d[2][29]), "+f"(d[2][30]), "+f"(d[2][31])
+               : "l"(adesc), "l"(bdesc));
+}
+__device__ __forceinline__ void wgmma_n256_f16(float (&d)[4][32], uint64_t adesc, uint64_t bdesc) {
+  asm volatile("{\n\t.reg .pred p;\n\tsetp.ne.b32 p, 1, 0;\n\twgmma.mma_async.sync.aligned.m64n256k16.f32.f16.f16 {%0, %1, %2, %3, %4, %5, %6, %7, %8, %9, %10, %11, %12, %13, %14, %15, %16, %17, %18, %19, %20, %21, %22, %23, %24, %25, %26, %27, %28, %29, %30, %31, %32, %33, %34, %35, %36, %37, %38, %39, %40, %41, %42, %43, %44, %45, %46, %47, %48, %49, %50, %51, %52, %53, %54, %55, %56, %57, %58, %59, %60, %61, %62, %63, %64, %65, %66, %67, %68, %69, %70, %71, %72, %73, %74, %75, %76, %77, %78, %79, %80, %81, %82, %83, %84, %85, %86, %87, %88, %89, %90, %91, %92, %93, %94, %95, %96, %97, %98, %99, %100, %101, %102, %103, %104, %105, %106, %107, %108, %109, %110, %111, %112, %113, %114, %115, %116, %117, %118, %119, %120, %121, %122, %123, %124, %125, %126, %127}, %128, %129, p, 1, 1, 0, 0;\n\t}"
+               : "+f"(d[0][0]), "+f"(d[0][1]), "+f"(d[0][2]), "+f"(d[0][3]), "+f"(d[0][4]), "+f"(d[0][5]), "+f"(d[0][6]), "+f"(d[0][7]), "+f"(d[0][8]), "+f"(d[0][9]), "+f"(d[0][10]), "+f"(d[0][11]), "+f"(d[0][12]), "+f"(d[0][13]), "+f"(d[0][14]), "+f"(d[0][15]), "+f"(d[0][16]), "+f"(d[0][17]), "+f"(d[0][18]), "+f"(d[0][19]), "+f"(d[0][20]), "+f"(d[0][21]), "+f"(d[0][22]), "+f"(d[0][23]), "+f"(d[0][24]), "+f"(d[0][25]), "+f"(d[0][26]), "+f"(d[0][27]), "+f"(d[0][28]), "+f"(d[0][29]), "+f"(d[0][30]), "+f"(d[0][31]), "+f"(d[1][0]), "+f"(d[1][1]), "+f"(d[1][2]), "+f"(d[1][3]), "+f"(d[1][4]), "+f"(d[1][5]), "+f"(d[1][6]), "+f"(d[1][7]), "+f"(d[1][8]), "+f"(d[1][9]), "+f"(d[1][10]), "+f"(d[1][11]), "+f"(d[1][12]), "+f"(d[1][13]), "+f"(d[1][14]), "+f"(d[1][15]), "+f"(d[1][16]), "+f"(d[1][17]), "+f"(d[1][18]), "+f"(d[1][19]), "+f"(d[1][20]), "+f"(d[1][21]), "+f"(d[1][22]), "+f"(d[1][23]), "+f"(d[1][24]), "+f"(d[1][25]), "+f"(d[1][26]), "+f"(d[1][27]), "+f"(d[1][28]), "+f"(d[1][29]), "+f"(d[1][30]), "+f"(d[1][31]), "+f"(d[2][0]), "+f"(d[2][1]), "+f"(d[2][2]), "+f"(d[2][3]), "+f"(d[2][4]), "+f"(d[2][5]), "+f"(d[2][6]), "+f"(d[2][7]), "+f"(d[2][8]), "+f"(d[2][9]), "+f"(d[2][10]), "+f"(d[2][11]), "+f"(d[2][12]), "+f"(d[2][13]), "+f"(d[2][14]), "+f"(d[2][15]), "+f"(d[2][16]), "+f"(d[2][17]), "+f"(d[2][18]), "+f"(d[2][19]), "+f"(d[2][20]), "+f"(d[2][21]), "+f"(d[2][22]), "+f"(d[2][23]), "+f"(d[2][24]), "+f"(d[2][25]), "+f"(d[2][26]), "+f"(d[2][27]), "+f"(d[2][28]), "+f"(d[2][29]), "+f"(d[2][30]), "+f"(d[2][31]), "+f"(d[3][0]), "+f"(d[3][1]), "+f"(d[3][2]), "+f"(d[3][3]), "+f"(d[3][4]), "+f"(d[3][5]), "+f"(d[3][6]), "+f"(d[3][7]), "+f"(d[3][8]), "+f"(d[3][9]), "+f"(d[3][10]), "+f"(d[3][11]), "+f"(d[3][12]), "+f"(d[3][13]), "+f"(d[3][14]), "+f"(d[3][15]), "+f"(d[3][16]), "+f"(d[3][17]), "+f"(d[3][18]), "+f"(d[3][19]), "+f"(d[3][20]), "+f"(d[3][21]), "+f"(d[3][22]), "+f"(d[3][23]), "+f"(d[3][24]), "+f"(d[3][25]), "+f"(d[3][26]), "+f"(d[3][27]), "+f"(d[3][28]), "+f"(d[3][29]), "+f"(d[3][30]), "+f"(d[3][31])
+               : "l"(adesc), "l"(bdesc));
+}
+__device__ __forceinline__ void wgmma_n256_bf16(float (&d)[4][32], uint64_t adesc, uint64_t bdesc) {
+  asm volatile("{\n\t.reg .pred p;\n\tsetp.ne.b32 p, 1, 0;\n\twgmma.mma_async.sync.aligned.m64n256k16.f32.bf16.bf16 {%0, %1, %2, %3, %4, %5, %6, %7, %8, %9, %10, %11, %12, %13, %14, %15, %16, %17, %18, %19, %20, %21, %22, %23, %24, %25, %26, %27, %28, %29, %30, %31, %32, %33, %34, %35, %36, %37, %38, %39, %40, %41, %42, %43, %44, %45, %46, %47, %48, %49, %50, %51, %52, %53, %54, %55, %56, %57, %58, %59, %60, %61, %62, %63, %64, %65, %66, %67, %68, %69, %70, %71, %72, %73, %74, %75, %76, %77, %78, %79, %80, %81, %82, %83, %84, %85, %86, %87, %88, %89, %90, %91, %92, %93, %94, %95, %96, %97, %98, %99, %100, %101, %102, %103, %104, %105, %106, %107, %108, %109, %110, %111, %112, %113, %114, %115, %116, %117, %118, %119, %120, %121, %122, %123, %124, %125, %126, %127}, %128, %129, p, 1, 1, 0, 0;\n\t}"
+               : "+f"(d[0][0]), "+f"(d[0][1]), "+f"(d[0][2]), "+f"(d[0][3]), "+f"(d[0][4]), "+f"(d[0][5]), "+f"(d[0][6]), "+f"(d[0][7]), "+f"(d[0][8]), "+f"(d[0][9]), "+f"(d[0][10]), "+f"(d[0][11]), "+f"(d[0][12]), "+f"(d[0][13]), "+f"(d[0][14]), "+f"(d[0][15]), "+f"(d[0][16]), "+f"(d[0][17]), "+f"(d[0][18]), "+f"(d[0][19]), "+f"(d[0][20]), "+f"(d[0][21]), "+f"(d[0][22]), "+f"(d[0][23]), "+f"(d[0][24]), "+f"(d[0][25]), "+f"(d[0][26]), "+f"(d[0][27]), "+f"(d[0][28]), "+f"(d[0][29]), "+f"(d[0][30]), "+f"(d[0][31]), "+f"(d[1][0]), "+f"(d[1][1]), "+f"(d[1][2]), "+f"(d[1][3]), "+f"(d[1][4]), "+f"(d[1][5]), "+f"(d[1][6]), "+f"(d[1][7]), "+f"(d[1][8]), "+f"(d[1][9]), "+f"(d[1][10]), "+f"(d[1][11]), "+f"(d[1][12]), "+f"(d[1][13]), "+f"(d[1][14]), "+f"(d[1][15]), "+f"(d[1][16]), "+f"(d[1][17]), "+f"(d[1][18]), "+f"(d[1][19]), "+f"(d[1][20]), "+f"(d[1][21]), "+f"(d[1][22]), "+f"(d[1][23]), "+f"(d[1][24]), "+f"(d[1][25]), "+f"(d[1][26]), "+f"(d[1][27]), "+f"(d[1][28]), "+f"(d[1][29]), "+f"(d[1][30]), "+f"(d[1][31]), "+f"(d[2][0]), "+f"(d[2][1]), "+f"(d[2][2]), "+f"(d[2][3]), "+f"(d[2][4]), "+f"(d[2][5]), "+f"(d[2][6]), "+f"(d[2][7]), "+f"(d[2][8]), "+f"(d[2][9]), "+f"(d[2][10]), "+f"(d[2][11]), "+f"(d[2][12]), "+f"(d[2][13]), "+f"(d[2][14]), "+f"(d[2][15]), "+f"(d[2][16]), "+f"(d[2][17]), "+f"(d[2][18]), "+f"(d[2][19]), "+f"(d[2][20]), "+f"(d[2][21]), "+f"(d[2][22]), "+f"(d[2][23]), "+f"(d[2][24]), "+f"(d[2][25]), "+f"(d[2][26]), "+f"(d[2][27]), "+f"(d[2][28]), "+f"(d[2][29]), "+f"(d[2][30]), "+f"(d[2][31]), "+f"(d[3][0]), "+f"(d[3][1]), "+f"(d[3][2]), "+f"(d[3][3]), "+f"(d[3][4]), "+f"(d[3][5]), "+f"(d[3][6]), "+f"(d[3][7]), "+f"(d[3][8]), "+f"(d[3][9]), "+f"(d[3][10]), "+f"(d[3][11]), "+f"(d[3][12]), "+f"(d[3][13]), "+f"(d[3][14]), "+f"(d[3][15]), "+f"(d[3][16]), "+f"(d[3][17]), "+f"(d[3][18]), "+f"(d[3][19]), "+f"(d[3][20]), "+f"(d[3][21]), "+f"(d[3][22]), "+f"(d[3][23]), "+f"(d[3][24]), "+f"(d[3][25]), "+f"(d[3][26]), "+f"(d[3][27]), "+f"(d[3][28]), "+f"(d[3][29]), "+f"(d[3][30]), "+f"(d[3][31])
+               : "l"(adesc), "l"(bdesc));
+}
 GRL_WGMMA_RS(wgmma_rs_n32t_bf16, "bf16")
 GRL_WGMMA_RS(wgmma_rs_n32t_f16, "f16")
 
```
